# isunLt/U2MKD

Measured on AMD Instinct MI355X. Metric: LiDAR points/sec/node fwd+bwd (teacher+student+KD), 1/2/4/8 MI355X, higher is better.
Workload: dtype f32 (fp32 products emulated on the 16-bit matrix pipe: f16x2 forward / input gradient, bf16x3 weight gradient; fp32 accumulate)

## Files before the change

include/u2mkd_hip.h:

```cpp
#ifndef U2MKD_HIP_H
#define U2MKD_HIP_H

#include <stddef.h>
#include <stdint.h>

#ifdef __cplusplus
extern "C" {
#endif

typedef void *u2mkd_stream_t;

int u2mkd_version(void);
const char *u2mkd_last_error(void);
int u2mkd_stream_wait_stream(u2mkd_stream_t waiter, u2mkd_stream_t signaler);
void *u2mkd_mailbox_alloc(size_t bytes);
int u2mkd_mailbox_free(void *p);
int u2mkd_mailbox_post(const void *const *srcs, uint32_t is64, int32_t n, int64_t *slot, int64_t seq, u2mkd_stream_t s);

int u2mkd_hash(const int32_t *coords , int64_t n, int64_t *out , u2mkd_stream_t s);
int u2mkd_kernel_hash(const int32_t *coords , const int32_t *offsets , int64_t n,
                      int32_t k, int64_t *out , u2mkd_stream_t s);

size_t u2mkd_hash_table_bytes(int64_t n_refs);
int u2mkd_hash_table_build(const int64_t *refs, int64_t n_refs, void *table, u2mkd_stream_t s);
int u2mkd_hash_table_query(const void *table, int64_t n_refs, const int64_t *queries, int64_t n_q,
                           int64_t *out , u2mkd_stream_t s);
int u2mkd_hash_table_query2(const void *table, int64_t n_refs, const int64_t *queries, int64_t n_q, int64_t *out,
                            int32_t *out32, u2mkd_stream_t s);

int u2mkd_kmap_build_table(const void *table, int64_t n_refs, const int32_t *out_coords ,
                           int64_t n_out, const int32_t *offsets , int32_t k,
                           int32_t *nbr , u2mkd_stream_t s);
int u2mkd_kmap_invert(const int32_t *nbr , int64_t n_out, int32_t k, int64_t n_in,
                      int32_t *nbr_inv , u2mkd_stream_t s);
int u2mkd_kmap_sizes(const int32_t *nbr, int64_t n_out, int32_t k, int32_t *nbsizes ,
                     int32_t *block_counts , u2mkd_stream_t s);
int u2mkd_kmap_compact(const int32_t *nbr, int64_t n_out, int32_t k, const int32_t *nbsizes ,
                       int32_t *block_counts ,
                       int32_t *nbmaps , u2mkd_stream_t s);

int64_t u2mkd_pairs_capacity(int64_t n_in, int64_t n_out, int32_t k);
int u2mkd_pairs_build(const int32_t *nbr , int64_t n_out, int64_t n_in, int32_t k,
                      const int32_t *nbsizes, int32_t *block_counts, int32_t *pair_in, int32_t *pair_out,
                      int32_t *pos_out, int32_t *pos_in, int32_t *tile_k, int32_t *meta, u2mkd_stream_t s);
int u2mkd_downsample_keys(const int32_t *coords , int64_t n, int32_t sx, int32_t sy, int32_t sz,
                          int64_t *keys , u2mkd_stream_t s);
int u2mkd_downsample_keys_checked(const int32_t *coords , int64_t n, int32_t sx, int32_t sy, int32_t sz,
                                  int64_t *keys , int32_t *range_flag, u2mkd_stream_t s);
int u2mkd_unpack_keys(const int64_t *keys, int64_t n, int32_t *coords , u2mkd_stream_t s);
int u2mkd_downsample_keys_general(const int32_t *coords , int64_t n, int32_t tsx, int32_t tsy, int32_t tsz, int32_t kx,
                                  int32_t ky, int32_t kz, int32_t sx, int32_t sy, int32_t sz, const int32_t *cmin ,
                                  int32_t m, int64_t *keys , int32_t *range_flag, u2mkd_stream_t s);
int u2mkd_floor_coords(const float *pc , int64_t n, int32_t stride, int32_t *out , u2mkd_stream_t s);

int u2mkd_transpose_weights(const float *w , int32_t k, int32_t cin, int32_t cout,
                            float *wt , u2mkd_stream_t s);
int u2mkd_conv_forward(const float *in , int64_t n_in, int32_t cin, const float *wt ,
                       int32_t cout, const int32_t *nbr , int64_t n_out, int32_t k, int32_t kflip,
                       float *out , u2mkd_stream_t s);
int u2mkd_conv_forward_sorted(const float *in, int64_t n_in, int32_t cin, const float *wt, int32_t cout,
                              const int32_t *nbr_sorted , const int32_t *order ,
                              const int32_t *tile_order , int64_t n_out, int32_t k,
                              int32_t kflip, float *out , u2mkd_stream_t s);
int32_t u2mkd_conv_lk_supported(int32_t cin, int32_t cout, int32_t k);
int u2mkd_conv_forward_lk(const float *in , int64_t n_in, int32_t cin, const float *wt ,
                          int32_t cout, const int32_t *nbr , int64_t ld, int64_t n_rows, int32_t k, int32_t kflip,
                          float *out , u2mkd_stream_t s);
int32_t u2mkd_conv_tiles_supported(int32_t cin, int32_t cout, int32_t k);
int32_t u2mkd_conv_tiles_arith(int32_t cin, int32_t cout, int32_t k);
size_t u2mkd_weight_fragments_bytes(int32_t k, int32_t rows, int32_t cols, int32_t arith);
int u2mkd_weight_fragments(const float *w, int32_t k, int32_t rows, int32_t cols, int32_t transpose, int32_t arith,
                           void *wf, u2mkd_stream_t s);
int u2mkd_weight_fragments_batch(const int64_t *jobs, int32_t n_jobs, int64_t total_units, u2mkd_stream_t s);
int u2mkd_conv_forward_tiles(const float *in, int64_t n_in, int32_t cin, const void *wf, int32_t cout,
                             const int32_t *nbr_sorted , const int32_t *order ,
                             const int32_t *items ,
                             const int32_t *n_items , int64_t n_out, int32_t k,
                             int32_t kflip, int32_t arith, float *out , u2mkd_stream_t s);
int u2mkd_conv_forward_tiles_ep(const float *in, int64_t n_in, int32_t cin, const void *wf, int32_t cout,
                                const int32_t *nbr_sorted, const int32_t *order, const int32_t *items,
                                const int32_t *n_items, int64_t n_out, int32_t k, int32_t kflip, int32_t arith,
                                const float *scale , const float *shift , const float *res ,
                                int32_t relu, float *out, u2mkd_stream_t s);
int32_t u2mkd_pairs_gather_sum_stats_slab_rows(void);
int32_t u2mkd_pairs_gather_sum_stats_supported(int32_t cout);
int u2mkd_pairs_gather_sum_stats(const float *y, const int32_t *pos, int64_t n_rows, int32_t k, int32_t cout, float *out,
                                 float *partial, u2mkd_stream_t s);
int u2mkd_pairs_gather_sum_ep(const float *y, const int32_t *pos, int64_t n_rows, int32_t k, int32_t cout, const float *scale,
                              const float *shift, const float *res, int32_t relu, float *out, u2mkd_stream_t s);
int u2mkd_debug_conv_forward_sorted(const float *in, int64_t n_in, int32_t cin, const float *wt, int32_t cout,
                                    const int32_t *nbr_sorted, const int32_t *order, const int32_t *tile_order,
                                    int64_t n_out, int32_t k, int32_t kflip, int32_t variant, float *out,
                                    u2mkd_stream_t s);
int u2mkd_debug_conv_tile_pairs_stamps(const float *in, int64_t n_in, const void *wf ,
                                       const int32_t *nbr_sorted, const int32_t *order, const int32_t *items,
                                       const int32_t *n_items, int64_t n_out, int32_t k, int32_t arith, float *out,
                                       uint64_t *stamps, u2mkd_stream_t s);
int u2mkd_debug_wgrad_stamps(const float *a, const float *b, const int32_t *pairs, const int32_t *plan, int64_t n_rows,
                             int32_t k, void *workspace, uint64_t *stamps, u2mkd_stream_t s);
int u2mkd_conv_forward_pairs(const float *in, int64_t n_in, int32_t cin, const float *wt, int32_t cout,
                             const int32_t *pair_idx, const int32_t *tile_k, const int32_t *meta, int64_t capacity,
                             int32_t k, int32_t kc, float *y , u2mkd_stream_t s);
int32_t u2mkd_conv_pairs_x3_supported(int32_t cin, int32_t cout);
int u2mkd_conv_forward_pairs_x3(const float *in, int64_t n_in, int32_t cin, const void *wf, int32_t cout,
                                const int32_t *pair_idx, const int32_t *tile_k, const int32_t *meta, int64_t capacity,
                                int32_t k, float *y , u2mkd_stream_t s);
int u2mkd_linear_forward(const float *x , int64_t n, int32_t cin, const float *w , int32_t cout,
                         const float *bias , int32_t kc, float *y, u2mkd_stream_t s);
int u2mkd_linear_forward_x3(const float *x , int64_t n, int32_t cin, const void *wf, int32_t cout,
                            const float *bias , float *y , u2mkd_stream_t s);
int32_t u2mkd_conv_pairs_f16x2_supported(int32_t cin, int32_t cout);
int u2mkd_conv_forward_pairs_f16x2(const float *in, int64_t n_in, int32_t cin, const void *wf, int32_t cout,
                                    const int32_t *pair_idx, const int32_t *tile_k, const int32_t *meta, int64_t capacity,
                                    int32_t k, float *y, u2mkd_stream_t s);
int u2mkd_linear_forward_f16x2(const float *x, int64_t n, int32_t cin, const void *wf, int32_t cout, const float *bias,
                               float *y, u2mkd_stream_t s);
int u2mkd_pairs_gather_sum(const float *y, const int32_t *pos , int64_t n_rows, int32_t k, int32_t cout,
                           float *out , u2mkd_stream_t s);
int u2mkd_kmap_rowmask(const int32_t *nbr , int64_t n_out, int32_t k, int32_t *mask ,
                       u2mkd_stream_t s);
int u2mkd_conv_forward_tiles_bf16(const void *in , int64_t n_in, int32_t cin, const void *wf, int32_t cout,
                                  const int32_t *nbr_sorted, const int32_t *order, const int32_t *items,
                                  const int32_t *n_items, int64_t n_out, int32_t k, int32_t kflip,
                                  void *out , u2mkd_stream_t s);
int u2mkd_conv_wgrad_pairs_bf16(const void *a , int32_t ca, const void *b , int32_t cb,
                                const int32_t *pairs, const int32_t *plan, int64_t n_rows, int32_t k, int32_t swap,
                                void *workspace, size_t workspace_bytes, float *dw , u2mkd_stream_t s);
int u2mkd_conv_forward_tiles_f16(const void *in , int64_t n_in, int32_t cin, const void *wf, int32_t cout,
                                 const int32_t *nbr_sorted, const int32_t *order, const int32_t *items,
                                 const int32_t *n_items, int64_t n_out, int32_t k, int32_t kflip,
                                 void *out , u2mkd_stream_t s);
int u2mkd_conv_wgrad_pairs_f16(const void *a , int32_t ca, const void *b , int32_t cb,
                               const int32_t *pairs, const int32_t *plan, int64_t n_rows, int32_t k, int32_t swap,
                               void *workspace, size_t workspace_bytes, float *dw , u2mkd_stream_t s);
int u2mkd_conv_forward_pairs_f16(const void *in , int64_t n_in, int32_t cin, const void *wf, int32_t cout,
                                  const int32_t *pair_idx, const int32_t *tile_k, const int32_t *meta, int64_t capacity,
                                  int32_t k, void *y , u2mkd_stream_t s);
int u2mkd_linear_forward_f16(const void *x , int64_t n, int32_t cin, const void *wf, int32_t cout,
                             const float *bias , void *y , u2mkd_stream_t s);
int u2mkd_pairs_gather_sum_f16(const void *y , const int32_t *pos , int64_t n_rows, int32_t k,
                               int32_t cout, void *out , u2mkd_stream_t s);
int u2mkd_conv_forward_pairs_bf16(const void *in , int64_t n_in, int32_t cin, const void *wf, int32_t cout,
                                   const int32_t *pair_idx, const int32_t *tile_k, const int32_t *meta, int64_t capacity,
                                   int32_t k, void *y , u2mkd_stream_t s);
int u2mkd_linear_forward_bf16(const void *x , int64_t n, int32_t cin, const void *wf, int32_t cout,
                              const float *bias , void *y , u2mkd_stream_t s);
int u2mkd_pairs_gather_sum_bf16(const void *y , const int32_t *pos , int64_t n_rows, int32_t k,
                                int32_t cout, void *out , u2mkd_stream_t s);
size_t u2mkd_tile_schedule_workspace_bytes(int64_t n_rows);
int u2mkd_tile_schedule(const int32_t *mask , const int32_t *order , int64_t n_rows,
                        int32_t k, int32_t split0, int32_t split1, void *workspace, int32_t *tile_order,
                        int32_t *items, int32_t *n_items, u2mkd_stream_t s);
int32_t u2mkd_wgrad_plan_ints(int32_t k);
int u2mkd_wgrad_plan(const int32_t *nbsizes , int32_t k, int64_t n_rows, int32_t *plan, u2mkd_stream_t s);
size_t u2mkd_conv_wgrad_pairs_workspace_bytes(int64_t n_rows, int32_t ca, int32_t cb, int32_t k);
int u2mkd_conv_wgrad_pairs(const float *a, int32_t ca, const float *b, int32_t cb, const int32_t *pairs ,
                           const int32_t *plan, int64_t n_rows, int32_t k, int32_t swap, void *workspace,
                           size_t workspace_bytes, float *dw , u2mkd_stream_t s);

size_t u2mkd_convolution_workspace_bytes(int64_t n_in_rows, int64_t n_out_rows, int32_t cin, int32_t cout,
                                         const int32_t *nbsizes_host , int32_t k);
int u2mkd_convolution_forward(const float *in_feat , int64_t n_in_rows, int32_t cin,
                              float *out_feat , int64_t n_out_rows, int32_t cout,
                              const float *kernel , const int32_t *nbmaps ,
                              const int32_t *nbsizes_host , int32_t k, int32_t transpose, void *workspace,
                              size_t workspace_bytes, u2mkd_stream_t s);
int u2mkd_convolution_backward(const float *in_feat , int64_t n_in_rows, int32_t cin,
                               float *grad_in_feat , const float *grad_out_feat ,
                               int64_t n_out_rows, int32_t cout, const float *kernel ,
                               float *grad_kernel , const int32_t *nbmaps, const int32_t *nbsizes_host,
                               int32_t k, int32_t transpose, void *workspace, size_t workspace_bytes, u2mkd_stream_t s);

int u2mkd_count(const int32_t *idx , int64_t n, int32_t *counts , int64_t num,
                u2mkd_stream_t s);
int u2mkd_voxelize_forward(const float *feats , const int32_t *idx , const int32_t *counts ,
                           int64_t n, int64_t nv, int32_t c, float *out , u2mkd_stream_t s);
int u2mkd_voxelize_backward(const float *grad_out , const int32_t *idx, const int32_t *counts, int64_t n,
                            int64_t nv, int32_t c, float *grad_feats , u2mkd_stream_t s);
int u2mkd_devoxelize_forward(const float *feats , const int32_t *idx , const float *w ,
                             int64_t n, int32_t c, float *out , u2mkd_stream_t s);
int u2mkd_devoxelize_backward(const float *grad_out , const int32_t *idx , const float *w ,
                              int64_t n, int64_t nv, int32_t c, float *grad_feats ,
                              u2mkd_stream_t s);
int u2mkd_segment_sum(const float *src , int32_t c, const int32_t *entry_row ,
                      const float *entry_w , const int32_t *seg_offsets , int64_t nv,
                      int32_t mean, float *out , u2mkd_stream_t s);
int u2mkd_segment_mean(const float *src , int32_t c, const int32_t *entry_row ,
                       const int32_t *seg_offsets , const int32_t *counts , int64_t nv,
                       float *out , u2mkd_stream_t s);
int u2mkd_segment_mean_bf16(const void *src , int32_t c, const int32_t *entry_row ,
                            const int32_t *seg_offsets , const int32_t *counts , int64_t nv,
                            void *out , u2mkd_stream_t s);
int u2mkd_segment_mean_f16(const void *src , int32_t c, const int32_t *entry_row ,
                           const int32_t *seg_offsets , const int32_t *counts , int64_t nv,
                           void *out , u2mkd_stream_t s);
int u2mkd_voxelize_backward_bf16(const void *grad_out , const int32_t *idx, const int32_t *counts, int64_t n,
                                 int64_t nv, int32_t c, void *grad_feats , u2mkd_stream_t s);
int u2mkd_devoxelize_forward_bf16(const void *feats , const int32_t *idx , const float *w ,
                                  int64_t n, int32_t c, void *out , u2mkd_stream_t s);
int u2mkd_segment_sum_bf16(const void *src , int32_t c, const int32_t *entry_row ,
                           const float *entry_w , const int32_t *seg_offsets , int64_t nv,
                           int32_t mean, void *out , u2mkd_stream_t s);
int u2mkd_voxelize_backward_f16(const void *grad_out , const int32_t *idx, const int32_t *counts, int64_t n,
                                int64_t nv, int32_t c, void *grad_feats , u2mkd_stream_t s);
int u2mkd_devoxelize_forward_f16(const void *feats , const int32_t *idx , const float *w ,
                                 int64_t n, int32_t c, void *out , u2mkd_stream_t s);
int u2mkd_segment_sum_f16(const void *src , int32_t c, const int32_t *entry_row ,
                          const float *entry_w , const int32_t *seg_offsets , int64_t nv,
                          int32_t mean, void *out , u2mkd_stream_t s);
size_t u2mkd_csr_workspace_bytes(int64_t n_entries, int64_t nv);
int u2mkd_csr_build(const int32_t *keys , int64_t n_entries, int64_t nv, void *workspace,
                    int32_t *order , int32_t *seg , u2mkd_stream_t s);
size_t u2mkd_devoxelize_plan_workspace_bytes(int64_t n, int64_t nv);
int u2mkd_devoxelize_plan(const int32_t *idx8 , const float *w8 , int64_t n, int64_t nv, void *workspace,
                          int32_t *entry_row , float *entry_w , int32_t *seg , u2mkd_stream_t s);
int u2mkd_ti_weights(const float *coords , const int64_t *idx_kn , int64_t n,
                     float scale, float *w_n8 , int32_t *idx_n8 , u2mkd_stream_t s);

int u2mkd_up_plan(const int32_t *idx8 , int64_t n, int32_t H, int32_t W, int32_t h, int32_t w, float rh, float rw,
                  int32_t *idx_out , float *w_out , u2mkd_stream_t s);
int u2mkd_upbn_stats(const float *x, int32_t n_img, int32_t c, int32_t h, int32_t w, const float *a, const float *b,
                     const float *ay, const float *ax, int32_t rows_per_chunk, float *partial, u2mkd_stream_t s);
int u2mkd_upbn_dense_grad(const float *x, int32_t n_img, int32_t c, int32_t h, int32_t w, const float *a, const float *b,
                          const float *ay, const float *ax, const float *c0 , const float *c1 ,
                          int32_t rows_per_chunk, float *dx, u2mkd_stream_t s);

int u2mkd_up_bilinear_forward(const float *x, const float *skip , int64_t planes, int32_t h, int32_t w, int32_t H,
                              int32_t W, float rh, float rw, float *y, u2mkd_stream_t s);
int u2mkd_up_bilinear_backward(const float *g, int64_t planes, int32_t h, int32_t w, int32_t H, int32_t W, const int32_t *taps_y,
                               const float *wy, const int32_t *taps_x, const float *wx, int32_t tiled, float *dx, u2mkd_stream_t s);

int u2mkd_maxpool3s2_forward(const float *x, int64_t planes, int32_t h, int32_t w, float *y, uint8_t *code, u2mkd_stream_t s);
int u2mkd_maxpool3s2_backward(const float *dy, const uint8_t *code, int64_t planes, int32_t h, int32_t w, float *dx,
                              u2mkd_stream_t s);

int u2mkd_transpose_batched(const float *in, float *out, int32_t batch, int32_t rows, int32_t cols, u2mkd_stream_t s);
int u2mkd_transpose_batched_scaled(const float *in, float *out, int32_t batch, int32_t rows, int32_t cols, float scale,
                                   u2mkd_stream_t s);

int u2mkd_l2c_combine_forward(const float *g0, const float *g1, const float *g2, const float *g3, int32_t n_grids, int32_t n_img,
                              int32_t h, int32_t w, int32_t c, int32_t ch1, int32_t cw1, int32_t ch2, int32_t cw2, int32_t ch3,
                              int32_t cw3, float *out_rows, u2mkd_stream_t s);
int u2mkd_l2c_combine_backward(const float *g_rows, int32_t n_img, int32_t h, int32_t w, int32_t c, int32_t ch, int32_t cw,
                               float *d_grid, u2mkd_stream_t s);

int32_t u2mkd_select_mse_partials(void);
int u2mkd_select_mse_forward(const float *gathered, const float *pseudo, const uint8_t *fov, int64_t n, int32_t c, float *out,
                             float *partial, float *stats, u2mkd_stream_t s);
int u2mkd_select_mse_backward(const float *g_out, const float *g_loss, const float *stats, const float *gathered,
                              const float *pseudo, const uint8_t *fov, int64_t n, int32_t c, float *d_gathered, float *d_pseudo,
                              u2mkd_stream_t s);
int u2mkd_lovasz_errors(const float *probas, const int64_t *labels, int32_t ignore_index, int64_t n, int32_t c, float *errors,
                        double *keys, u2mkd_stream_t s);
int u2mkd_lovasz_gather(const int64_t *perm, const int64_t *labels, int32_t ignore_index, int64_t n, int32_t c,
                        int32_t *fg_sorted, u2mkd_stream_t s);
int64_t u2mkd_lovasz_partials(int64_t n, int32_t c);
int u2mkd_lovasz_terms(const int64_t *perm, const float *errors, const int64_t *csum, const int32_t *fg_sorted, int64_t n,
                       int32_t c, float *jgrad, float *partial, float *stats, u2mkd_stream_t s);
int u2mkd_lovasz_backward(const float *g_out, const float *stats, const int64_t *perm, const float *jgrad, const float *probas,
                          const int64_t *labels, int32_t ignore_index, int64_t n, int32_t c, float *d_probas, u2mkd_stream_t s);
int64_t u2mkd_ce_partials(int64_t n);
int u2mkd_ce_forward(const float *x, const int64_t *labels, int32_t ignore_index, int64_t n, int32_t c, float *lse, float *partial,
                     float *stats, u2mkd_stream_t s);
int u2mkd_ce_backward(const float *g_out, const float *stats, const float *x, const float *lse, const int64_t *labels,
                      int32_t ignore_index, int64_t n, int32_t c, float *dx, u2mkd_stream_t s);
int u2mkd_kl_forward(const float *s_logits, const float *t_logits, const int64_t *t_index, int64_t n, int32_t c, float *rows,
                     float *partial, float *stats, u2mkd_stream_t s);
int u2mkd_kl_backward(const float *g_out, const float *s_logits, const float *t_logits, const int64_t *t_index, const float *rows,
                      int64_t n, int32_t c, float *ds, u2mkd_stream_t s);
int u2mkd_c2l_plan(const float *pixel_coords, const uint8_t *mask, int32_t ncam, int64_t n, int32_t sample, int32_t h,
                   int32_t w, int32_t *idx8 , float *w8 , u2mkd_stream_t s);
int u2mkd_l2c_keys(const float *pixel_coords, const uint8_t *mask, int32_t ncam, int64_t n, int32_t sample, int64_t row0,
                   int64_t e0, int32_t ch, int32_t cw, int32_t *pix, int32_t *key_d, int32_t *key_s, int32_t *row,
                   u2mkd_stream_t s);
int u2mkd_l2c_finish(const int32_t *order_d, const int32_t *seg_d, const int32_t *order_s, const int32_t *pix,
                     const int32_t *row, int64_t n_entries, int32_t *fwd_row, float *fwd_w, int32_t *bwd_pix, float *bwd_w,
                     u2mkd_stream_t s);

int64_t u2mkd_bn_num_slabs(int64_t n);
int u2mkd_bn_train_forward(const void *x, const void *res, int32_t row_dtype, int64_t n, int32_t c, const float *gamma,
                           const float *beta, float eps, float momentum, float *running_mean, float *running_var,
                           int64_t *num_batches_tracked, int32_t relu, float *partial, float *mean ,
                           float *invstd , void *y, u2mkd_stream_t s);
int u2mkd_bn_train_forward_from_partial(const float *x, const float *res, int64_t n, int32_t c, const float *gamma,
                                        const float *beta, float eps, float momentum, float *running_mean, float *running_var,
                                        int64_t *num_batches_tracked, int32_t relu, const float *partial, int32_t slab_rows,
                                        float *mean , float *invstd , float *y, u2mkd_stream_t s);
int u2mkd_bn_eval_forward(const void *x, const void *res, int32_t row_dtype, int64_t n, int32_t c, const float *gamma,
                          const float *beta, float eps, const float *running_mean, const float *running_var, int32_t relu,
                          float *invstd , void *y, u2mkd_stream_t s);
int u2mkd_bn_backward(const void *dy, const void *x, const void *res, int32_t row_dtype, int64_t n, int32_t c,
                      const float *mean, const float *invstd, const float *gamma, const float *beta, int32_t relu,
                      int32_t training, float *partial, float *dgamma , float *dbeta , void *dx, void *dres,
                      u2mkd_stream_t s);

int u2mkd_bn_local_stats(const void *x, int32_t row_dtype, int64_t n, int32_t c, float *partial ,
                         float *stats , u2mkd_stream_t s);
int u2mkd_bn_merge_stats(const float *gathered , int32_t world, int32_t c, float eps, float momentum,
                         float *running_mean, float *running_var, float *mean , float *invstd ,
                         float *total , int64_t *num_batches_tracked, u2mkd_stream_t s);
int u2mkd_bn_apply(const void *x, const void *res, int32_t row_dtype, int64_t n, int32_t c, const float *mean,
                   const float *invstd, const float *gamma, const float *beta, int32_t relu, void *y, u2mkd_stream_t s);
int u2mkd_bn_backward_local(const void *dy, const void *x, const void *res, int32_t row_dtype, int64_t n, int32_t c,
                            const float *mean, const float *invstd, const float *gamma, const float *beta, int32_t relu,
                            float *partial , float *sums , float *keep ,
                            u2mkd_stream_t s);
int u2mkd_bn_backward_apply(const void *dy, const void *x, const void *res, int32_t row_dtype, int64_t n, int32_t c,
                            const float *total_n , const float *mean, const float *invstd, const float *gamma,
                            const float *beta, int32_t relu, const float *sums , void *dx, void *dres,
                            u2mkd_stream_t s);

int64_t u2mkd_ln_num_slabs(int64_t n, int32_t c);
int u2mkd_ln_forward(const void *x, int32_t row_dtype, int64_t n, int32_t c, const float *gamma, const float *beta, float eps,
                     float *mean , float *rstd , void *y, u2mkd_stream_t s);
int u2mkd_ln_add_forward(const void *a, const void *b, const float *w , int32_t row_dtype, int64_t n,
                         int32_t c, const float *gamma, const float *beta, float eps, float *mean ,
                         float *rstd , void *stream_out, void *y, u2mkd_stream_t s);
int u2mkd_ln_backward(const void *dy, const void *x, const void *ds , const float *w ,
                      int32_t row_dtype, int64_t n, int32_t c, const float *mean, const float *rstd, const float *gamma,
                      float *partial , float *dgamma , float *dbeta , void *dx,
                      void *db , u2mkd_stream_t s);

int64_t u2mkd_scene_num_slabs(int64_t n, int64_t nb);
int u2mkd_scene_slabs(const int32_t *seg , int64_t nb, int64_t n, int32_t *slab_seg ,
                      int32_t *slabs , int64_t nslab, u2mkd_stream_t s);
int u2mkd_gn_forward(const void *x, int32_t row_dtype, int64_t n, int32_t c, int32_t groups, const int32_t *bidx,
                     const int32_t *order, const int32_t *seg, const int32_t *slab_seg, const int32_t *slabs, int64_t nslab,
                     int64_t nb, const float *gamma, const float *beta, float eps, void *partial, float *mean, float *rstd,
                     void *y, u2mkd_stream_t s);
int u2mkd_gn_backward(const void *dy, const void *x, int32_t row_dtype, int64_t n, int32_t c, int32_t groups, const int32_t *bidx,
                      const int32_t *order, const int32_t *seg, const int32_t *slab_seg, const int32_t *slabs, int64_t nslab,
                      int64_t nb, const float *mean, const float *rstd, const float *gamma, float *partial, float *sums,
                      float *dgamma, float *dbeta, void *dx, u2mkd_stream_t s);
int u2mkd_scene_pool_forward(const void *x, int32_t row_dtype, int64_t n, int32_t c, int32_t mode, const int32_t *order,
                             const int32_t *seg, const int32_t *slab_seg, const int32_t *slabs, int64_t nslab, int64_t nb,
                             void *partial, float *out, int32_t *arg, u2mkd_stream_t s);
int u2mkd_scene_pool_backward(const float *dy, int32_t row_dtype, int64_t n, int32_t c, int32_t mode, const int32_t *bidx,
                              const int32_t *seg, const int32_t *arg, int64_t nb, void *dx, u2mkd_stream_t s);

int u2mkd_bev_plan(const int32_t *coords, int64_t n, int32_t dim, int32_t mode, int32_t hmode, int32_t s0, int32_t s1, int32_t s2,
                   int32_t a0, int32_t a1, int32_t a2, int32_t h, int32_t w, int32_t nz, int64_t *keys ,
                   int32_t *hidx , int32_t *block , u2mkd_stream_t s);
int u2mkd_bev_tables(const int32_t *group, const int32_t *hidx, int64_t n_in, int64_t n_out, int32_t nk, int32_t *nbr,
                     int32_t *nbr_inv, u2mkd_stream_t s);
int u2mkd_bev_segment_mean(const void *src, int32_t row_dtype, int64_t n_src, int32_t c, const int32_t *order, const int32_t *seg,
                           int64_t nv, void *out, u2mkd_stream_t s);
int u2mkd_bev_dense_store(const void *src, int32_t row_dtype, int64_t n_rows, int32_t c, const int32_t *seg, const int32_t *order,
                          int64_t nb, int32_t z, int32_t h, int32_t w, void *out, u2mkd_stream_t s);
int u2mkd_bev_dense_gather(const void *dout, int32_t row_dtype, int64_t n_rows, int32_t c, const int32_t *seg, const int32_t *order,
                           int64_t nb, int32_t z, int32_t h, int32_t w, void *dsrc, u2mkd_stream_t s);

int u2mkd_sptr_window_keys(const float *xyz , const int32_t *batch , int64_t n, const float *lo4,
                           const float *hi4, float sx, float sy, float sz, int64_t *keys , u2mkd_stream_t s);
size_t u2mkd_sptr_plan_prepare_workspace_bytes(void);
int u2mkd_sptr_plan_prepare(const float *xyz , const int32_t *batch , int64_t n, float cx, float cy, float cz,
                            float sx, float sy, float sz, float *sphere, float *bounds, int64_t *keys_cubic,
                            int64_t *keys_sphere, void *workspace, u2mkd_stream_t s);
int u2mkd_sptr_window_ranges(const int64_t *sorted_keys, int64_t n, int32_t *wstart , int32_t *wlen ,
                             u2mkd_stream_t s);
int u2mkd_sptr_quant_coords(const float *xyz , const int32_t *sort_idx , int64_t n, const float *lo,
                            float wx, float wy, float wz, float qx, float qy, float qz, int32_t *qc ,
                            float *radial , u2mkd_stream_t s);
int u2mkd_sptr_attention_forward(const float *q, const float *k, const float *v, const int32_t *sort_idx,
                                 const int32_t *wstart, const int32_t *wlen, const int32_t *qc, const float *radial,
                                 const float *tq, const float *tk, const float *tv, int32_t L, int32_t qgl,
                                 float split_a, int64_t n, int32_t h, int32_t hdim, float *out, float *lse,
                                 u2mkd_stream_t s);
size_t u2mkd_sptr_backward_workspace_bytes(int64_t n, int32_t h, int32_t L);
int u2mkd_sptr_attention_backward(const float *q, const float *k, const float *v, const float *out, const float *dout,
                                  const float *lse, const int32_t *sort_idx, const int32_t *wstart,
                                  const int32_t *wlen, const int32_t *qc, const float *radial, const float *tq,
                                  const float *tk, const float *tv, int32_t L, int32_t qgl, float split_a,
                                  int32_t qc_span, int64_t n, int32_t h, int32_t hdim, float *delta ,
                                  void *workspace, size_t workspace_bytes, float *dq, float *dk, float *dv, float *dtq,
                                  float *dtk, float *dtv, u2mkd_stream_t s);
int u2mkd_sptr_attention_forward_strided(const float *q, const float *k, const float *v, int64_t ld_qkv, float q_scale,
                                         const int32_t *sort_idx, const int32_t *wstart, const int32_t *wlen,
                                         const int32_t *qc, const float *radial, const float *tq, const float *tk,
                                         const float *tv, int32_t L, int32_t qgl, float split_a, int64_t n, int32_t h,
                                         int32_t hdim, float *out, int64_t ld_out, float *lse, u2mkd_stream_t s);
int u2mkd_sptr_attention_backward_strided(const float *q, const float *k, const float *v, int64_t ld_qkv, float q_scale,
                                          const float *out, const float *dout, int64_t ld_out, const float *lse,
                                          const int32_t *sort_idx, const int32_t *wstart, const int32_t *wlen,
                                          const int32_t *qc, const float *radial, const float *tq, const float *tk,
                                          const float *tv, int32_t L, int32_t qgl, float split_a, int32_t qc_span,
                                          int64_t n, int32_t h, int32_t hdim, float *delta ,
                                          void *workspace, size_t workspace_bytes, float *dq, float *dk, float *dv,
                                          int64_t ld_grad, float *dtq, float *dtk, float *dtv, u2mkd_stream_t s);
#include "u2mkd_hip_sptr_rows16.h"

int u2mkd_sptr_table_reduce(const void *workspace, int64_t n, int32_t h, int32_t L, float split_a, float *dtq, float *dtk,
                            float *dtv, u2mkd_stream_t s);

int u2mkd_sptr_quant_coords_shifted(const float *xyz , const int32_t *sort_idx , int64_t n, const float *lo,
                                    float wx, float wy, float wz, float shx, float shy, float shz, float qx, float qy,
                                    float qz, int32_t *qc , float *radial , u2mkd_stream_t s);

int u2mkd_sptr_plain_forward_strided(const float *q, const float *k, const float *v, int64_t ld_qkv, float q_scale,
                                     const int32_t *sort_idx, const int32_t *wstart, const int32_t *wlen, int64_t n,
                                     int32_t h, int32_t hdim, float *out, int64_t ld_out, float *lse, u2mkd_stream_t s);
int u2mkd_sptr_plain_backward_strided(const float *q, const float *k, const float *v, int64_t ld_qkv, float q_scale,
                                      const float *out, const float *dout, int64_t ld_out, const float *lse,
                                      const int32_t *sort_idx, const int32_t *wstart, const int32_t *wlen, int64_t n,
                                      int32_t h, int32_t hdim, float *delta , float *dq, float *dk,
                                      float *dv, int64_t ld_grad, u2mkd_stream_t s);

int u2mkd_sptr_precompute_all(int32_t N, int32_t n, uint32_t n_max, const int32_t *counts, const int32_t *offsets,
                              const int32_t *sq_offsets, int32_t *index_0_offsets, int32_t *index_1_offsets,
                              int32_t *index_0, int32_t *index_1, u2mkd_stream_t s);
int u2mkd_sptr_attention_step1_forward(int32_t N_q, int32_t N_k, int32_t M, int32_t h, int32_t hdim, uint32_t n_max,
                                       const float *q, const float *k, const int32_t *index0, const int32_t *index1,
                                       float *attn, u2mkd_stream_t s);
int u2mkd_sptr_attention_step1_backward(int32_t N, int32_t M, int32_t h, int32_t hdim, uint32_t n_max,
                                        const float *grad_out, const int32_t *index0, const int32_t *index0_offsets,
                                        const int32_t *index1, const int32_t *index1_offsets, const float *q,
                                        const float *k, float *grad_q, float *grad_k, u2mkd_stream_t s);
int u2mkd_sptr_attention_step2_forward(int32_t N, int32_t M, int32_t h, int32_t hdim, int32_t n_max, const float *attn,
                                       const float *v, const int32_t *index0_offsets, const int32_t *index1,
                                       float *output, u2mkd_stream_t s);
int u2mkd_sptr_attention_step2_backward(int32_t N, int32_t M, int32_t h, int32_t hdim, int32_t n_max,
                                        const float *grad_out, const int32_t *index0, const int32_t *index0_offsets,
                                        const int32_t *index1, const int32_t *index1_offsets, const float *attn,
                                        const float *v, float *grad_attn, float *grad_v, u2mkd_stream_t s);
int u2mkd_sptr_dot_prod_with_idx_forward(int32_t N, int32_t M, int32_t h, int32_t hdim, int32_t n_max, int32_t L,
                                         const float *q, const int32_t *index_q, const int32_t *index_q_offsets,
                                         const float *k, const int32_t *index_k, const float *table_q,
                                         const float *table_k, const int32_t *rel_idx, float *output,
                                         u2mkd_stream_t s);
int u2mkd_sptr_dot_prod_with_idx_all_forward(int32_t N, int32_t M, int32_t h, int32_t hdim, int32_t n_max, int32_t L,
                                             const float *q, const int32_t *index_q, const int32_t *index_q_offsets,
                                             const float *k, const int32_t *index_k, const float *table_q,
                                             const float *table_k, const int32_t *rel_idx, float *output,
                                             u2mkd_stream_t s);
int u2mkd_sptr_dot_prod_with_idx_backward(int32_t N, int32_t M, int32_t h, int32_t hdim, int32_t n_max, int32_t L,
                                          const float *grad_out, const float *q, const int32_t *index_q_offsets,
                                          const float *k, const int32_t *index_k_offsets, const int32_t *index_k,
                                          const float *table_q, const float *table_k, const int32_t *rel_idx,
                                          float *grad_q, float *grad_k, float *grad_table_q, float *grad_table_k,
                                          u2mkd_stream_t s);
int u2mkd_sptr_attention_step2_with_rel_pos_value_forward(int32_t N, int32_t M, int32_t h, int32_t hdim, int32_t n_max,
                                                          const float *attn, const float *v,
                                                          const int32_t *index0_offsets, const int32_t *index1,
                                                          const float *table, const int32_t *rel_idx, float *output,
                                                          u2mkd_stream_t s);
int u2mkd_sptr_attention_step2_with_rel_pos_value_backward(int32_t N, int32_t M, int32_t h, int32_t hdim, int32_t L,
                                                           int32_t n_max, const float *grad_out, const int32_t *index0,
                                                           const int32_t *index0_offsets, const int32_t *index1,
                                                           const int32_t *index1_offsets, const float *attn,
                                                           const float *v, const float *table, const int32_t *rel_idx,
                                                           float *grad_attn, float *grad_v, float *grad_table,
                                                           u2mkd_stream_t s);

size_t u2mkd_bn2d_workspace_bytes(int64_t b, int32_t c, int64_t hw);
int u2mkd_bn2d_train_forward(const float *x, const float *res, int64_t b, int32_t c, int64_t hw, const float *gamma,
                             const float *beta, float eps, float momentum, int32_t relu, float *running_mean,
                             float *running_var, int64_t *num_batches_tracked, void *workspace,
                             float *mean , float *invstd , float *y, u2mkd_stream_t s);
int u2mkd_bn2d_eval_forward(const float *x, const float *res, int64_t b, int32_t c, int64_t hw, const float *gamma,
                            const float *beta, float eps, int32_t relu, const float *running_mean,
                            const float *running_var, float *y, u2mkd_stream_t s);
int u2mkd_bn2d_backward(const float *dy, const float *x, const float *res, int64_t b, int32_t c, int64_t hw,
                        const float *mean, const float *invstd, const float *gamma, const float *beta, int32_t relu,
                        int32_t batch_stats, void *workspace, float *dgamma, float *dbeta, float *dx,
                        float *dres , u2mkd_stream_t s);

int u2mkd_bn2d_local_stats(const float *x, int64_t b, int32_t c, int64_t hw, void *workspace, float *stats ,
                           u2mkd_stream_t s);
int u2mkd_bn2d_apply(const float *x, const float *res, int64_t b, int32_t c, int64_t hw, const float *mean,
                     const float *invstd, const float *gamma, const float *beta, int32_t relu, float *y, u2mkd_stream_t s);
int u2mkd_bn2d_backward_local(const float *dy, const float *x, const float *res, int64_t b, int32_t c, int64_t hw,
                              const float *mean, const float *invstd, const float *gamma, const float *beta, int32_t relu,
                              void *workspace, float *sums , float *keep ,
                              u2mkd_stream_t s);
int u2mkd_bn2d_backward_apply(const float *dy, const float *x, const float *res, int64_t b, int32_t c, int64_t hw,
                              const float *total_n , const float *mean, const float *invstd, const float *gamma,
                              const float *beta, int32_t relu, const float *sums , float *dx,
                              float *dres , u2mkd_stream_t s);

size_t u2mkd_sptr_tiles_workspace_bytes(int64_t n, int32_t h);
int u2mkd_sptr_attention_forward_tiles(const float *q, const float *k, const float *v, int64_t ld_qkv, float q_scale,
                                       const int32_t *sort_idx, const int32_t *wstart, const int32_t *wlen, const int32_t *qc,
                                       const float *radial, const float *tq, const float *tk, const float *tv, int32_t L,
                                       int32_t qgl, float split_a, int64_t n, int32_t h, int32_t hdim, float *out, int64_t ld_out,
                                       float *lse, void *workspace, size_t workspace_bytes, u2mkd_stream_t s);

int32_t u2mkd_sgd_chunk_elements(void);
int u2mkd_sgd_batch(const int64_t *jobs, int32_t n_jobs, int64_t total_chunks, float lr, float momentum, float weight_decay,
                    int32_t nesterov, int32_t contract, u2mkd_stream_t s);
int u2mkd_grads_unscale_check(const int64_t *jobs, int32_t n_jobs, int64_t total_chunks, const float *inv_scale, float *found_inf,
                              u2mkd_stream_t s);
int u2mkd_sgd_batch_amp(const int64_t *jobs, int32_t n_jobs, int64_t total_chunks, float lr, float momentum, float weight_decay,
                        int32_t nesterov, int32_t contract, const float *grad_scale, const float *found_inf, u2mkd_stream_t s);
int u2mkd_adam_batch(const int64_t *jobs, int32_t n_jobs, int64_t total_chunks, const float *scalars, float decay, float weight_decay,
                     int32_t decoupled, float w1, float beta2, float w2, float eps, int32_t form, u2mkd_stream_t s);
int u2mkd_adam_batch_amp(const int64_t *jobs, int32_t n_jobs, int64_t total_chunks, const float *scalars, int32_t window, float decay,
                         float weight_decay, int32_t decoupled, float w1, float beta2, float w2, float eps, int32_t form,
                         const int32_t *count_in, int32_t *count_out, int32_t count_known, const float *grad_scale,
                         const float *found_inf, u2mkd_stream_t s);
int u2mkd_debug_adam_stage(int32_t stage, int32_t form, const float *a, const float *b, const float *c, float scalar, float *out,
                           int64_t n, u2mkd_stream_t s);

#ifdef __cplusplus
}
#endif
#endif
```

u2mkd_amd/_lib.py:

```python
from __future__ import annotations

import ctypes as C
import os

import torch

_HERE = os.path.dirname(os.path.abspath(__file__))
LIB_PATH = os.path.join(_HERE, 'lib', 'libu2mkd_hip%s.so' % os.environ.get('U2MKD_LIB_SUFFIX', ''))

_i32, _i64, _sz, _f32, _p = C.c_int32, C.c_int64, C.c_size_t, C.c_float, C.c_void_p

SIGNATURES = {
    'u2mkd_version': (C.c_int, []),
    'u2mkd_last_error': (C.c_char_p, []),
    'u2mkd_hash': (C.c_int, [_p, _i64, _p, _p]),
    'u2mkd_kernel_hash': (C.c_int, [_p, _p, _i64, _i32, _p, _p]),
    'u2mkd_hash_table_bytes': (_sz, [_i64]),
    'u2mkd_hash_table_build': (C.c_int, [_p, _i64, _p, _p]),
    'u2mkd_hash_table_query': (C.c_int, [_p, _i64, _p, _i64, _p, _p]),
    'u2mkd_hash_table_query2': (C.c_int, [_p, _i64, _p, _i64, _p, _p, _p]),
    'u2mkd_kmap_build_table': (C.c_int, [_p, _i64, _p, _i64, _p, _i32, _p, _p]),
    'u2mkd_kmap_invert': (C.c_int, [_p, _i64, _i32, _i64, _p, _p]),
    'u2mkd_kmap_sizes': (C.c_int, [_p, _i64, _i32, _p, _p, _p]),
    'u2mkd_kmap_compact': (C.c_int, [_p, _i64, _i32, _p, _p, _p, _p]),
    'u2mkd_downsample_keys': (C.c_int, [_p, _i64, _i32, _i32, _i32, _p, _p]),
    'u2mkd_downsample_keys_checked': (C.c_int, [_p, _i64, _i32, _i32, _i32, _p, _p, _p]),
    'u2mkd_downsample_keys_general': (C.c_int, [_p, _i64] + [_i32] * 9 + [_p, _i32, _p, _p, _p]),
    'u2mkd_floor_coords': (C.c_int, [_p, _i64, _i32, _p, _p]),
    'u2mkd_unpack_keys': (C.c_int, [_p, _i64, _p, _p]),
    'u2mkd_transpose_weights': (C.c_int, [_p, _i32, _i32, _i32, _p, _p]),
    'u2mkd_conv_forward': (C.c_int, [_p, _i64, _i32, _p, _i32, _p, _i64, _i32, _i32, _p, _p]),
    'u2mkd_conv_forward_sorted': (C.c_int, [_p, _i64, _i32, _p, _i32, _p, _p, _p, _i64, _i32, _i32, _p, _p]),
    'u2mkd_debug_conv_forward_sorted': (C.c_int, [_p, _i64, _i32, _p, _i32, _p, _p, _p, _i64, _i32, _i32, _i32, _p, _p]),
    'u2mkd_conv_lk_supported': (_i32, [_i32, _i32, _i32]),
    'u2mkd_conv_forward_lk': (C.c_int, [_p, _i64, _i32, _p, _i32, _p, _i64, _i64, _i32, _i32, _p, _p]),
    'u2mkd_stream_wait_stream': (C.c_int, [_p, _p]),
    'u2mkd_sgd_chunk_elements': (_i32, []),
    'u2mkd_sgd_batch': (C.c_int, [_p, _i32, _i64, _f32, _f32, _f32, _i32, _i32, _p]),
    'u2mkd_grads_unscale_check': (C.c_int, [_p, _i32, _i64, _p, _p, _p]),
    'u2mkd_sgd_batch_amp': (C.c_int, [_p, _i32, _i64, _f32, _f32, _f32, _i32, _i32, _p, _p, _p]),
    'u2mkd_adam_batch': (C.c_int, [_p, _i32, _i64, _p, _f32, _f32, _i32, _f32, _f32, _f32, _f32, _i32, _p]),
    'u2mkd_adam_batch_amp': (C.c_int, [_p, _i32, _i64, _p, _i32, _f32, _f32, _i32, _f32, _f32, _f32, _f32, _i32, _p, _p, _i32, _p, _p, _p]),
    'u2mkd_debug_adam_stage': (C.c_int, [_i32, _i32, _p, _p, _p, _f32, _p, _i64, _p]),
    'u2mkd_mailbox_alloc': (_p, [_sz]),
    'u2mkd_mailbox_free': (C.c_int, [_p]),
    'u2mkd_mailbox_post': (C.c_int, [_p, C.c_uint32, _i32, _p, _i64, _p]),
    'u2mkd_conv_tiles_supported': (_i32, [_i32, _i32, _i32]),
    'u2mkd_conv_tiles_arith': (_i32, [_i32, _i32, _i32]),
    'u2mkd_weight_fragments_bytes': (_sz, [_i32, _i32, _i32, _i32]),
    'u2mkd_weight_fragments': (C.c_int, [_p, _i32, _i32, _i32, _i32, _i32, _p, _p]),
    'u2mkd_weight_fragments_batch': (C.c_int, [_p, _i32, _i64, _p]),
    'u2mkd_conv_forward_tiles': (C.c_int, [_p, _i64, _i32, _p, _i32, _p, _p, _p, _p, _i64, _i32, _i32, _i32, _p, _p]),
    'u2mkd_conv_forward_tiles_ep': (C.c_int, [_p, _i64, _i32, _p, _i32, _p, _p, _p, _p, _i64, _i32, _i32, _i32, _p, _p, _p, _i32, _p, _p]),
    'u2mkd_pairs_gather_sum_ep': (C.c_int, [_p, _p, _i64, _i32, _i32, _p, _p, _p, _i32, _p, _p]),
    'u2mkd_pairs_gather_sum_stats_slab_rows': (_i32, []),
    'u2mkd_pairs_gather_sum_stats_supported': (_i32, [_i32]),
    'u2mkd_pairs_gather_sum_stats': (C.c_int, [_p, _p, _i64, _i32, _i32, _p, _p, _p]),
    'u2mkd_debug_conv_tile_pairs_stamps': (C.c_int, [_p, _i64, _p, _p, _p, _p, _p, _i64, _i32, _i32, _p, _p, _p]),
    'u2mkd_debug_wgrad_stamps': (C.c_int, [_p, _p, _p, _p, _i64, _i32, _p, _p, _p]),
    'u2mkd_conv_forward_pairs': (C.c_int, [_p, _i64, _i32, _p, _i32, _p, _p, _p, _i64, _i32, _i32, _p, _p]),
    'u2mkd_conv_pairs_x3_supported': (_i32, [_i32, _i32]),
    'u2mkd_conv_forward_pairs_x3': (C.c_int, [_p, _i64, _i32, _p, _i32, _p, _p, _p, _i64, _i32, _p, _p]),
    'u2mkd_linear_forward': (C.c_int, [_p, _i64, _i32, _p, _i32, _p, _i32, _p, _p]),
    'u2mkd_bn2d_workspace_bytes': (C.c_size_t, [_i64, _i32, _i64]),
    'u2mkd_bn2d_train_forward': (C.c_int, [_p, _p, _i64, _i32, _i64, _p, _p, C.c_float, C.c_float, _i32, _p, _p, _p, _p, _p, _p, _p, _p]),
    'u2mkd_bn2d_eval_forward': (C.c_int, [_p, _p, _i64, _i32, _i64, _p, _p, C.c_float, _i32, _p, _p, _p, _p]),
    'u2mkd_bn2d_backward': (C.c_int, [_p, _p, _p, _i64, _i32, _i64, _p, _p, _p, _p, _i32, _i32, _p, _p, _p, _p, _p, _p]),
    'u2mkd_bn2d_local_stats': (C.c_int, [_p, _i64, _i32, _i64, _p, _p, _p]),
    'u2mkd_bn2d_apply': (C.c_int, [_p, _p, _i64, _i32, _i64, _p, _p, _p, _p, _i32, _p, _p]),
    'u2mkd_bn2d_backward_local': (C.c_int, [_p, _p, _p, _i64, _i32, _i64, _p, _p, _p, _p, _i32, _p, _p, _p, _p]),
    'u2mkd_bn2d_backward_apply': (C.c_int, [_p, _p, _p, _i64, _i32, _i64, _p, _p, _p, _p, _p, _i32, _p, _p, _p, _p]),
    'u2mkd_linear_forward_x3': (C.c_int, [_p, _i64, _i32, _p, _i32, _p, _p, _p]),
    'u2mkd_conv_pairs_f16x2_supported': (_i32, [_i32, _i32]),
    'u2mkd_conv_forward_pairs_f16x2': (C.c_int, [_p, _i64, _i32, _p, _i32, _p, _p, _p, _i64, _i32, _p, _p]),
    'u2mkd_linear_forward_f16x2': (C.c_int, [_p, _i64, _i32, _p, _i32, _p, _p, _p]),
    'u2mkd_pairs_capacity': (_i64, [_i64, _i64, _i32]),
    'u2mkd_pairs_build': (C.c_int, [_p, _i64, _i64, _i32, _p, _p, _p, _p, _p, _p, _p, _p, _p]),
    'u2mkd_pairs_gather_sum': (C.c_int, [_p, _p, _i64, _i32, _i32, _p, _p]),
    'u2mkd_kmap_rowmask': (C.c_int, [_p, _i64, _i32, _p, _p]),
    'u2mkd_tile_schedule_workspace_bytes': (_sz, [_i64]),
    'u2mkd_tile_schedule': (C.c_int, [_p, _p, _i64, _i32, _i32, _i32, _p, _p, _p, _p, _p]),
    'u2mkd_wgrad_plan_ints': (_i32, [_i32]),
    'u2mkd_wgrad_plan': (C.c_int, [_p, _i32, _i64, _p, _p]),
    'u2mkd_conv_wgrad_pairs_workspace_bytes': (_sz, [_i64, _i32, _i32, _i32]),
    'u2mkd_conv_wgrad_pairs': (C.c_int, [_p, _i32, _p, _i32, _p, _p, _i64, _i32, _i32, _p, _sz, _p, _p]),
    'u2mkd_conv_forward_tiles_bf16': (C.c_int, [_p, _i64, _i32, _p, _i32, _p, _p, _p, _p, _i64, _i32, _i32, _p, _p]),
    'u2mkd_conv_forward_tiles_f16': (C.c_int, [_p, _i64, _i32, _p, _i32, _p, _p, _p, _p, _i64, _i32, _i32, _p, _p]),
    'u2mkd_conv_wgrad_pairs_bf16': (C.c_int, [_p, _i32, _p, _i32, _p, _p, _i64, _i32, _i32, _p, _sz, _p, _p]),
    'u2mkd_conv_wgrad_pairs_f16': (C.c_int, [_p, _i32, _p, _i32, _p, _p, _i64, _i32, _i32, _p, _sz, _p, _p]),
    'u2mkd_conv_forward_pairs_bf16': (C.c_int, [_p, _i64, _i32, _p, _i32, _p, _p, _p, _i64, _i32, _p, _p]),
    'u2mkd_conv_forward_pairs_f16': (C.c_int, [_p, _i64, _i32, _p, _i32, _p, _p, _p, _i64, _i32, _p, _p]),
    'u2mkd_linear_forward_bf16': (C.c_int, [_p, _i64, _i32, _p, _i32, _p, _p, _p]),
    'u2mkd_linear_forward_f16': (C.c_int, [_p, _i64, _i32, _p, _i32, _p, _p, _p]),
    'u2mkd_pairs_gather_sum_bf16': (C.c_int, [_p, _p, _i64, _i32, _i32, _p, _p]),
    'u2mkd_pairs_gather_sum_f16': (C.c_int, [_p, _p, _i64, _i32, _i32, _p, _p]),
    'u2mkd_convolution_workspace_bytes': (_sz, [_i64, _i64, _i32, _i32, _p, _i32]),
    'u2mkd_convolution_forward': (C.c_int, [_p, _i64, _i32, _p, _i64, _i32, _p, _p, _p, _i32, _i32, _p, _sz, _p]),
    'u2mkd_convolution_backward': (C.c_int, [_p, _i64, _i32, _p, _p, _i64, _i32, _p, _p, _p, _p, _i32, _i32, _p, _sz, _p]),
    'u2mkd_bn_num_slabs': (_i64, [_i64]),
    'u2mkd_bn_train_forward': (C.c_int, [_p, _p, _i32, _i64, _i32, _p, _p, _f32, _f32, _p, _p, _p, _i32, _p, _p, _p, _p, _p]),
    'u2mkd_bn_train_forward_from_partial': (C.c_int, [_p, _p, _i64, _i32, _p, _p, _f32, _f32, _p, _p, _p, _i32, _p, _i32, _p, _p, _p, _p]),
    'u2mkd_bn_eval_forward': (C.c_int, [_p, _p, _i32, _i64, _i32, _p, _p, _f32, _p, _p, _i32, _p, _p, _p]),
    'u2mkd_bn_backward': (C.c_int, [_p, _p, _p, _i32, _i64, _i32, _p, _p, _p, _p, _i32, _i32, _p, _p, _p, _p, _p, _p]),
    'u2mkd_bn_local_stats': (C.c_int, [_p, _i32, _i64, _i32, _p, _p, _p]),
    'u2mkd_bn_merge_stats': (C.c_int, [_p, _i32, _i32, _f32, _f32, _p, _p, _p, _p, _p, _p, _p]),
    'u2mkd_bn_apply': (C.c_int, [_p, _p, _i32, _i64, _i32, _p, _p, _p, _p, _i32, _p, _p]),
    'u2mkd_bn_backward_local': (C.c_int, [_p, _p, _p, _i32, _i64, _i32, _p, _p, _p, _p, _i32, _p, _p, _p, _p]),
    'u2mkd_bn_backward_apply': (C.c_int, [_p, _p, _p, _i32, _i64, _i32, _p, _p, _p, _p, _p, _i32, _p, _p, _p, _p]),
    'u2mkd_ln_num_slabs': (_i64, [_i64, _i32]),
    'u2mkd_ln_forward': (C.c_int, [_p, _i32, _i64, _i32, _p, _p, _f32, _p, _p, _p, _p]),
    'u2mkd_ln_add_forward': (C.c_int, [_p, _p, _p, _i32, _i64, _i32, _p, _p, _f32, _p, _p, _p, _p, _p]),
    'u2mkd_ln_backward': (C.c_int, [_p, _p, _p, _p, _i32, _i64, _i32, _p, _p, _p, _p, _p, _p, _p, _p, _p]),
    'u2mkd_scene_num_slabs': (_i64, [_i64, _i64]),
    'u2mkd_scene_slabs': (C.c_int, [_p, _i64, _i64, _p, _p, _i64, _p]),
    'u2mkd_gn_forward': (C.c_int, [_p, _i32, _i64, _i32, _i32, _p, _p, _p, _p, _p, _i64, _i64, _p, _p, _f32, _p, _p, _p, _p, _p]),
    'u2mkd_gn_backward': (C.c_int, [_p, _p, _i32, _i64, _i32, _i32, _p, _p, _p, _p, _p, _i64, _i64, _p, _p, _p, _p, _p, _p, _p, _p, _p]),
    'u2mkd_scene_pool_forward': (C.c_int, [_p, _i32, _i64, _i32, _i32, _p, _p, _p, _p, _i64, _i64, _p, _p, _p, _p]),
    'u2mkd_scene_pool_backward': (C.c_int, [_p, _i32, _i64, _i32, _i32, _p, _p, _p, _i64, _p, _p]),
    'u2mkd_bev_plan': (C.c_int, [_p, _i64] + [_i32] * 12 + [_p, _p, _p, _p]),
    'u2mkd_bev_tables': (C.c_int, [_p, _p, _i64, _i64, _i32, _p, _p, _p]),
    'u2mkd_bev_segment_mean': (C.c_int, [_p, _i32, _i64, _i32, _p, _p, _i64, _p, _p]),
    'u2mkd_bev_dense_store': (C.c_int, [_p, _i32, _i64, _i32, _p, _p, _i64, _i32, _i32, _i32, _p, _p]),
    'u2mkd_bev_dense_gather': (C.c_int, [_p, _i32, _i64, _i32, _p, _p, _i64, _i32, _i32, _i32, _p, _p]),
    'u2mkd_sptr_window_keys': (C.c_int, [_p, _p, _i64, _p, _p, _f32, _f32, _f32, _p, _p]),
    'u2mkd_select_mse_partials': (_i32, []),
    'u2mkd_select_mse_forward': (C.c_int, [_p, _p, _p, _i64, _i32, _p, _p, _p, _p]),
    'u2mkd_select_mse_backward': (C.c_int, [_p, _p, _p, _p, _p, _p, _i64, _i32, _p, _p, _p]),
    'u2mkd_sptr_plan_prepare_workspace_bytes': (_sz, []),
    'u2mkd_sptr_plan_prepare': (C.c_int, [_p, _p, _i64, _f32, _f32, _f32, _f32, _f32, _f32, _p, _p, _p, _p, _p, _p]),
    'u2mkd_sptr_window_ranges': (C.c_int, [_p, _i64, _p, _p, _p]),
    'u2mkd_sptr_quant_coords': (C.c_int, [_p, _p, _i64, _p, _f32, _f32, _f32, _f32, _f32, _f32, _p, _p, _p]),
    'u2mkd_sptr_attention_forward': (C.c_int, [_p, _p, _p, _p, _p, _p, _p, _p, _p, _p, _p, _i32, _i32, _f32, _i64, _i32, _i32, _p, _p, _p]),
    'u2mkd_sptr_backward_workspace_bytes': (_sz, [_i64, _i32, _i32]),
    'u2mkd_sptr_attention_backward': (C.c_int, [_p] * 14 + [_i32, _i32, _f32, _i32, _i64, _i32, _i32] + [_p, _p, _sz] + [_p] * 7),
    'u2mkd_sptr_tiles_workspace_bytes': (_sz, [_i64, _i32]),
    'u2mkd_sptr_attention_forward_tiles': (C.c_int, [_p, _p, _p, _i64, _f32] + [_p] * 8 + [_i32, _i32, _f32, _i64, _i32, _i32, _p, _i64, _p, _p, _sz, _p]),
    'u2mkd_sptr_attention_forward_strided': (C.c_int, [_p, _p, _p, _i64, _f32] + [_p] * 8 + [_i32, _i32, _f32, _i64, _i32, _i32, _p, _i64, _p, _p]),
    'u2mkd_sptr_attention_backward_strided': (C.c_int, [_p, _p, _p, _i64, _f32, _p, _p, _i64] + [_p] * 9 + [_i32, _i32, _f32, _i32, _i64, _i32, _i32]
                                              + [_p, _p, _sz] + [_p, _p, _p, _i64, _p, _p, _p, _p]),
    'u2mkd_sptr_table_reduce': (C.c_int, [_p, _i64, _i32, _i32, _f32, _p, _p, _p, _p]),
    'u2mkd_sptr_quant_coords_shifted': (C.c_int, [_p, _p, _i64, _p] + [_f32] * 9 + [_p, _p, _p]),
    'u2mkd_sptr_plain_forward_strided': (C.c_int, [_p, _p, _p, _i64, _f32, _p, _p, _p, _i64, _i32, _i32, _p, _i64, _p, _p]),
    'u2mkd_sptr_plain_backward_strided': (C.c_int, [_p, _p, _p, _i64, _f32, _p, _p, _i64, _p, _p, _p, _p, _i64, _i32, _i32,
                                                    _p, _p, _p, _p, _i64, _p]),
    'u2mkd_sptr_precompute_all': (C.c_int, [_i32, _i32, C.c_uint32] + [_p] * 8),
    'u2mkd_sptr_attention_step1_forward': (C.c_int, [_i32, _i32, _i32, _i32, _i32, C.c_uint32] + [_p] * 6),
    'u2mkd_sptr_attention_step1_backward': (C.c_int, [_i32, _i32, _i32, _i32, C.c_uint32] + [_p] * 10),
    'u2mkd_sptr_attention_step2_forward': (C.c_int, [_i32] * 5 + [_p] * 6),
    'u2mkd_sptr_attention_step2_backward': (C.c_int, [_i32] * 5 + [_p] * 10),
    'u2mkd_sptr_dot_prod_with_idx_forward': (C.c_int, [_i32] * 6 + [_p] * 10),
    'u2mkd_sptr_dot_prod_with_idx_all_forward': (C.c_int, [_i32] * 6 + [_p] * 10),
    'u2mkd_sptr_dot_prod_with_idx_backward': (C.c_int, [_i32] * 6 + [_p] * 14),
    'u2mkd_sptr_attention_step2_with_rel_pos_value_forward': (C.c_int, [_i32] * 5 + [_p] * 8),
    'u2mkd_sptr_attention_step2_with_rel_pos_value_backward': (C.c_int, [_i32] * 6 + [_p] * 13),
    'u2mkd_count': (C.c_int, [_p, _i64, _p, _i64, _p]),
    'u2mkd_voxelize_forward': (C.c_int, [_p, _p, _p, _i64, _i64, _i32, _p, _p]),
    'u2mkd_voxelize_backward': (C.c_int, [_p, _p, _p, _i64, _i64, _i32, _p, _p]),
    'u2mkd_devoxelize_forward': (C.c_int, [_p, _p, _p, _i64, _i32, _p, _p]),
    'u2mkd_devoxelize_backward': (C.c_int, [_p, _p, _p, _i64, _i64, _i32, _p, _p]),
    'u2mkd_segment_sum': (C.c_int, [_p, _i32, _p, _p, _p, _i64, _i32, _p, _p]),
    'u2mkd_voxelize_backward_bf16': (C.c_int, [_p, _p, _p, _i64, _i64, _i32, _p, _p]),
    'u2mkd_voxelize_backward_f16': (C.c_int, [_p, _p, _p, _i64, _i64, _i32, _p, _p]),
    'u2mkd_devoxelize_forward_bf16': (C.c_int, [_p, _p, _p, _i64, _i32, _p, _p]),
    'u2mkd_devoxelize_forward_f16': (C.c_int, [_p, _p, _p, _i64, _i32, _p, _p]),
    'u2mkd_segment_sum_bf16': (C.c_int, [_p, _i32, _p, _p, _p, _i64, _i32, _p, _p]),
    'u2mkd_segment_sum_f16': (C.c_int, [_p, _i32, _p, _p, _p, _i64, _i32, _p, _p]),
    'u2mkd_segment_mean': (C.c_int, [_p, _i32, _p, _p, _p, _i64, _p, _p]),
    'u2mkd_segment_mean_bf16': (C.c_int, [_p, _i32, _p, _p, _p, _i64, _p, _p]),
    'u2mkd_segment_mean_f16': (C.c_int, [_p, _i32, _p, _p, _p, _i64, _p, _p]),
    'u2mkd_c2l_plan': (C.c_int, [_p, _p, _i32, _i64, _i32, _i32, _i32, _p, _p, _p]),
    'u2mkd_l2c_keys': (C.c_int, [_p, _p, _i32, _i64, _i32, _i64, _i64, _i32, _i32, _p, _p, _p, _p, _p]),
    'u2mkd_l2c_finish': (C.c_int, [_p, _p, _p, _p, _p, _i64, _p, _p, _p, _p, _p]),
    'u2mkd_up_bilinear_forward': (C.c_int, [_p, _p, _i64, _i32, _i32, _i32, _i32, _f32, _f32, _p, _p]),
    'u2mkd_up_bilinear_backward': (C.c_int, [_p, _i64, _i32, _i32, _i32, _i32, _p, _p, _p, _p, _i32, _p, _p]),
    'u2mkd_maxpool3s2_forward': (C.c_int, [_p, _i64, _i32, _i32, _p, _p, _p]),
    'u2mkd_maxpool3s2_backward': (C.c_int, [_p, _p, _i64, _i32, _i32, _p, _p]),
    'u2mkd_transpose_batched': (C.c_int, [_p, _p, _i32, _i32, _i32, _p]),
    'u2mkd_transpose_batched_scaled': (C.c_int, [_p, _p, _i32, _i32, _i32, C.c_float, _p]),
    'u2mkd_l2c_combine_forward': (C.c_int, [_p, _p, _p, _p] + [_i32] * 11 + [_p, _p]),
    'u2mkd_l2c_combine_backward': (C.c_int, [_p] + [_i32] * 6 + [_p, _p]),
    'u2mkd_up_plan': (C.c_int, [_p, _i64, _i32, _i32, _i32, _i32, _f32, _f32, _p, _p, _p]),
    'u2mkd_upbn_stats': (C.c_int, [_p, _i32, _i32, _i32, _i32, _p, _p, _p, _p, _i32, _p, _p]),
    'u2mkd_upbn_dense_grad': (C.c_int, [_p, _i32, _i32, _i32, _i32, _p, _p, _p, _p, _p, _p, _i32, _p, _p]),
    'u2mkd_csr_workspace_bytes': (_sz, [_i64, _i64]),
    'u2mkd_lovasz_errors': (C.c_int, [_p, _p, _i32, _i64, _i32, _p, _p, _p]),
    'u2mkd_lovasz_gather': (C.c_int, [_p, _p, _i32, _i64, _i32, _p, _p]),
    'u2mkd_lovasz_partials': (_i64, [_i64, _i32]),
    'u2mkd_lovasz_terms': (C.c_int, [_p, _p, _p, _p, _i64, _i32, _p, _p, _p, _p]),
    'u2mkd_ce_partials': (_i64, [_i64]),
    'u2mkd_ce_forward': (C.c_int, [_p, _p, _i32, _i64, _i32, _p, _p, _p, _p]),
    'u2mkd_ce_backward': (C.c_int, [_p, _p, _p, _p, _p, _i32, _i64, _i32, _p, _p]),
    'u2mkd_kl_forward': (C.c_int, [_p, _p, _p, _i64, _i32, _p, _p, _p, _p]),
    'u2mkd_kl_backward': (C.c_int, [_p, _p, _p, _p, _p, _i64, _i32, _p, _p]),
    'u2mkd_lovasz_backward': (C.c_int, [_p, _p, _p, _p, _p, _p, _i32, _i64, _i32, _p, _p]),
    'u2mkd_csr_build': (C.c_int, [_p, _i64, _i64, _p, _p, _p, _p]),
    'u2mkd_devoxelize_plan_workspace_bytes': (C.c_size_t, [_i64, _i64]),
    'u2mkd_devoxelize_plan': (C.c_int, [_p, _p, _i64, _i64, _p, _p, _p, _p, _p]),
    'u2mkd_ti_weights': (C.c_int, [_p, _p, _i64, _f32, _p, _p, _p]),
}

SPTR_ROWS16_SIGNATURES = {
    name + sfx: SIGNATURES[name]
    for name in ('u2mkd_sptr_attention_forward_strided', 'u2mkd_sptr_attention_backward_strided') for sfx in ('_bf16', '_f16')}

_lib = None
_raw_stream = torch._C._cuda_getCurrentRawStream
_current_device = torch._C._cuda_getDevice


def load():
    global _lib
    if _lib is not None:
        return _lib
    if not os.path.exists(LIB_PATH):
        raise RuntimeError(
            f'{LIB_PATH} is missing: build it with `python -m u2mkd_amd.build` '
            '(u2mkd_amd has no CPU or PyTorch fallback path)')
    lib = C.CDLL(LIB_PATH)
    for name, (res, args) in list(SIGNATURES.items()) + list(SPTR_ROWS16_SIGNATURES.items()):
        fn = getattr(lib, name)
        fn.restype = res
        fn.argtypes = args
    _lib = lib
    return lib


def stream() -> int:
    return _raw_stream(_current_device())


def ptr(t):
    if t is None:
        return None
    return t.data_ptr()


_fns = {}


def call(name: str, *args):
    fn = _fns.get(name)
    if fn is None:
        fn = _fns[name] = getattr(load(), name)
    rc = fn(*args)
    if rc != 0:
        msg = load().u2mkd_last_error().decode('utf-8', 'replace')
        raise RuntimeError(f'{name} failed (rc={rc}): {msg}')


def require_cuda(*tensors):
    for t in tensors:
        if t is not None and not t.is_cuda:
            raise RuntimeError('u2mkd_amd operators run on the HIP device only (got a CPU tensor); '
                               'there is no CPU fallback')
```

u2mkd_amd/camera.py:

```python
import os

import torch
import torch.nn.functional as F
from torch import nn

__all__ = ['SwiftNetRes18', 'SwiftNetResNet', 'BNReluConv', 'BatchNorm2d', 'SyncBatchNorm2d', 'bn_act']

_HIP_BN2D = os.environ.get('U2MKD_BN2D', '1') != '0'


class _MaxPool3s2Function(torch.autograd.Function):
    @staticmethod
    def forward(ctx, x):
        from . import _lib as L
        n, c, h, w = x.shape
        oh, ow = (h - 1) // 2 + 1, (w - 1) // 2 + 1
        y = torch.empty(n, c, oh, ow, dtype=torch.float32, device=x.device)
        code = torch.empty(n, c, oh, ow, dtype=torch.uint8, device=x.device)
        L.call('u2mkd_maxpool3s2_forward', L.ptr(x), n * c, h, w, L.ptr(y), L.ptr(code), L.stream())
        ctx.save_for_backward(code)
        ctx.shape = (n, c, h, w)
        return y

    @staticmethod
    @torch.autograd.function.once_differentiable
    def backward(ctx, g):
        from . import _lib as L
        code, = ctx.saved_tensors
        n, c, h, w = ctx.shape
        dx = torch.empty(n, c, h, w, dtype=torch.float32, device=g.device)
        L.call('u2mkd_maxpool3s2_backward', L.ptr(g.contiguous()), L.ptr(code), n * c, h, w, L.ptr(dx), L.stream())
        return dx


class MaxPool3x3s2(nn.MaxPool2d):

    def __init__(self):
        super().__init__(kernel_size=3, stride=2, padding=1)

    def forward(self, x):
        if (x.is_cuda and x.dtype == torch.float32 and x.dim() == 4 and x.is_contiguous() and x.numel() and not torch.is_autocast_enabled()
                and x.shape[0] * x.shape[1] <= 65535 and x.shape[2] * x.shape[3] < 2 ** 31):
            return _MaxPool3s2Function.apply(x)
        return super().forward(x)


_UP_TAPS = {}
_UP_MODE = os.environ.get('U2MKD_UP_BILINEAR', '1')
_UP_HIP = None if _UP_MODE == 'auto' else _UP_MODE != '0'


def _up_on_hip():
    return torch.are_deterministic_algorithms_enabled() if _UP_HIP is None else _UP_HIP


def _up_taps(n_in, n_out, device):
    key = (n_in, n_out, str(device))
    if key not in _UP_TAPS:
        import numpy as np
        r = np.float32(n_in - 1) / np.float32(n_out - 1) if n_out > 1 else np.float32(0)
        src = (r * np.arange(n_out, dtype=np.float32)).astype(np.float32)
        i0 = src.astype(np.int64)
        ip = (i0 < n_in - 1).astype(np.int64)
        l1 = (src - i0.astype(np.float32)).astype(np.float32)
        l0 = (np.float32(1) - l1).astype(np.float32)
        first = np.full(n_in, n_out, np.int64)
        last = np.full(n_in, -1, np.int64)
        for idx in (i0, i0 + ip):
            np.minimum.at(first, idx, np.arange(n_out))
            np.maximum.at(last, idx, np.arange(n_out))
        cnt = np.maximum(last - first + 1, 0)
        ok = int(cnt.max()) <= 8
        taps = wts = span = None
        if ok:
            w = np.zeros((n_in, 8), np.float32)
            for o in range(n_out):
                w[i0[o], o - first[i0[o]]] += l0[o]
                w[i0[o] + ip[o], o - first[i0[o] + ip[o]]] += l1[o]
            first = np.where(cnt > 0, first, 0)
            span = {t: 1 << 30 if int(cnt.min()) == 0 else max(int(first[min(a + t, n_in) - 1] + cnt[min(a + t, n_in) - 1] - first[a]) for a in range(0, n_in, t))
                    for t in (16, 64)}
            taps = torch.tensor(np.stack([first, cnt], 1), dtype=torch.int32, device=device).contiguous()
            wts = torch.tensor(w, dtype=torch.float32, device=device).contiguous()
        _UP_TAPS[key] = (float(r), taps, wts, span)
    return _UP_TAPS[key]


class _UpBilinearFunction(torch.autograd.Function):

    @staticmethod
    def forward(ctx, x, skip, size):
        from . import _lib as L
        n, c, h, w = x.shape
        big_h, big_w = size
        rh, ty, wy, span_y = _up_taps(h, big_h, x.device)
        rw, tx, wx, span_x = _up_taps(w, big_w, x.device)
        y = torch.empty(n, c, big_h, big_w, dtype=torch.float32, device=x.device)
        L.call('u2mkd_up_bilinear_forward', L.ptr(x), L.ptr(skip), n * c, h, w, big_h, big_w, rh, rw, L.ptr(y), L.stream())
        tiled = int(span_y[16] <= 40 and span_x[64] <= 136 and n * c <= 65535)
        ctx.geom = (n, c, h, w, big_h, big_w, ty, wy, tx, wx, tiled)
        ctx.has_skip = skip is not None
        return y

    @staticmethod
    @torch.autograd.function.once_differentiable
    def backward(ctx, g):
        from . import _lib as L
        n, c, h, w, big_h, big_w, ty, wy, tx, wx, tiled = ctx.geom
        g = g.contiguous()
        dx = None
        if ctx.needs_input_grad[0]:
            dx = torch.empty(n, c, h, w, dtype=torch.float32, device=g.device)
            L.call('u2mkd_up_bilinear_backward', L.ptr(g), n * c, h, w, big_h, big_w, L.ptr(ty), L.ptr(wy), L.ptr(tx), L.ptr(wx),
                   tiled, L.ptr(dx), L.stream())
        return dx, (g if ctx.has_skip and ctx.needs_input_grad[1] else None), None


def _up(x, size, skip=None):
    size = tuple(int(v) for v in size)
    if (_up_on_hip() and x.is_cuda and x.dtype == torch.float32 and x.dim() == 4 and x.is_contiguous() and x.numel() and not torch.is_autocast_enabled()
            and x.shape[0] * x.shape[1] <= 65535 and size[0] >= x.shape[2] and size[1] >= x.shape[3] and (skip is None or (skip.dtype == x.dtype and skip.is_contiguous()
                                                                                      and skip.shape[2:] == size))):
        if _up_taps(x.shape[2], size[0], x.device)[1] is not None and _up_taps(x.shape[3], size[1], x.device)[1] is not None:
            return _UpBilinearFunction.apply(x, skip, size)
    y = F.interpolate(x, size, mode='bilinear', align_corners=True)
    return y if skip is None else y + skip


class _BatchNorm2dFunction(torch.autograd.Function):

    @staticmethod
    def forward(ctx, x, weight, bias, res, bn, relu):
        from . import _lib as L
        b, c, h, w = x.shape
        hw = h * w
        y = torch.empty_like(x)
        st = L.stream()
        batch_stats = bn.training or bn.running_mean is None
        if batch_stats:
            ws = torch.empty(max(L.load().u2mkd_bn2d_workspace_bytes(b, c, hw), 16), dtype=torch.uint8, device=x.device)
            mean = torch.empty(c, dtype=torch.float32, device=x.device)
            invstd = torch.empty_like(mean)
            track = bn.training and bn.running_mean is not None
            L.call('u2mkd_bn2d_train_forward', L.ptr(x), L.ptr(res), b, c, hw, L.ptr(weight), L.ptr(bias), bn.eps,
                   bn.momentum if track else 0.0, int(relu), L.ptr(bn.running_mean if track else None),
                   L.ptr(bn.running_var if track else None), L.ptr(bn.num_batches_tracked if track else None),
                   L.ptr(ws), L.ptr(mean), L.ptr(invstd), L.ptr(y), st)
            if track:
                torch._C._increment_version([t for t in (bn.running_mean, bn.running_var, bn.num_batches_tracked) if t is not None])
        else:
            mean, invstd = bn.running_mean, torch.rsqrt(bn.running_var + bn.eps)
            L.call('u2mkd_bn2d_eval_forward', L.ptr(x), L.ptr(res), b, c, hw, L.ptr(weight), L.ptr(bias), bn.eps, int(relu),
                   L.ptr(bn.running_mean), L.ptr(bn.running_var), L.ptr(y), st)
        ctx.save_for_backward(x, weight, bias, res, mean, invstd)
        ctx.relu, ctx.batch_stats = bool(relu), batch_stats
        return y

    @staticmethod
    def backward(ctx, dy):
        from . import _lib as L
        x, weight, bias, res, mean, invstd = ctx.saved_tensors
        b, c, h, w = x.shape
        hw = h * w
        dy = dy.contiguous()
        dx = torch.empty_like(x)
        dres = torch.empty_like(x) if res is not None else None
        dgamma = torch.empty(c, dtype=torch.float32, device=x.device)
        dbeta = torch.empty_like(dgamma)
        ws = torch.empty(max(L.load().u2mkd_bn2d_workspace_bytes(b, c, hw), 16), dtype=torch.uint8, device=x.device)
        L.call('u2mkd_bn2d_backward', L.ptr(dy), L.ptr(x), L.ptr(res), b, c, hw, L.ptr(mean), L.ptr(invstd), L.ptr(weight),
               L.ptr(bias), int(ctx.relu), int(ctx.batch_stats), L.ptr(ws), L.ptr(dgamma), L.ptr(dbeta), L.ptr(dx), L.ptr(dres),
               L.stream())
        return dx, (dgamma if weight is not None else None), (dbeta if bias is not None else None), dres, None, None


class BatchNorm2d(nn.BatchNorm2d):

    def forward(self, x, relu=False, residual=None):
        if (_HIP_BN2D and x.is_cuda and x.dtype == torch.float32 and x.dim() == 4 and x.is_contiguous() and x.numel() > 0
                and not torch.is_autocast_enabled() and (self.momentum is not None or not self.training)
                and (residual is None or (residual.dtype == x.dtype and residual.shape == x.shape))):
            if residual is not None:
                residual = residual.contiguous()
            return _BatchNorm2dFunction.apply(x, self.weight, self.bias, residual, self, relu)
        y = super().forward(x)
        if residual is not None:
            y = y + residual
        return F.relu(y) if relu else y


class _SyncBatchNorm2dFunction(torch.autograd.Function):

    @staticmethod
    def forward(ctx, x, weight, bias, res, bn, relu, group, world):
        from . import _lib as L
        from .torchsparse.nn.functional import _gather_rows, note_collective
        b, c, h, w = x.shape
        hw = h * w
        dev, st = x.device, L.stream()
        ws = torch.empty(max(L.load().u2mkd_bn2d_workspace_bytes(b, c, hw), 16), dtype=torch.uint8, device=dev)
        stats = torch.empty(2 * c + 1, dtype=torch.float32, device=dev)
        L.call('u2mkd_bn2d_local_stats', L.ptr(x), b, c, hw, L.ptr(ws), L.ptr(stats), st)
        note_collective('all_gather', stats)
        if world > 1:
            gathered = torch.empty(world, 2 * c + 1, dtype=torch.float32, device=dev)
            _gather_rows(gathered, stats, group)
        else:
            gathered = stats.view(1, -1)
        mit = torch.empty(2 * c + 1, dtype=torch.float32, device=dev)
        mean, invstd, total = mit[:c], mit[c:2 * c], mit[2 * c:]
        track = bn.running_mean is not None
        L.call('u2mkd_bn_merge_stats', L.ptr(gathered), world, c, float(bn.eps), float(bn.momentum if track else 0.0),
               L.ptr(bn.running_mean if track else None), L.ptr(bn.running_var if track else None), L.ptr(mean),
               L.ptr(invstd), L.ptr(total), L.ptr(bn.num_batches_tracked if track else None), L.stream())
        if track:
            torch._C._increment_version([t for t in (bn.running_mean, bn.running_var, bn.num_batches_tracked) if t is not None])
        y = torch.empty_like(x)
        L.call('u2mkd_bn2d_apply', L.ptr(x), L.ptr(res), b, c, hw, L.ptr(mean), L.ptr(invstd), L.ptr(weight), L.ptr(bias),
               int(relu), L.ptr(y), L.stream())
        ctx.save_for_backward(x, weight, bias, res, mean, invstd, total)
        ctx.relu, ctx.group, ctx.world = bool(relu), group, world
        return y

    @staticmethod
    def backward(ctx, dy):
        from . import _lib as L
        from .torchsparse.nn.functional import _sum_over_ranks, note_collective
        x, weight, bias, res, mean, invstd, total = ctx.saved_tensors
        b, c, h, w = x.shape
        hw = h * w
        dy = dy.contiguous()
        dev = x.device
        ws = torch.empty(max(L.load().u2mkd_bn2d_workspace_bytes(b, c, hw), 16), dtype=torch.uint8, device=dev)
        both = torch.empty(2, 2 * c, dtype=torch.float32, device=dev)
        sums, local = both[0], both[1]
        L.call('u2mkd_bn2d_backward_local', L.ptr(dy), L.ptr(x), L.ptr(res), b, c, hw, L.ptr(mean), L.ptr(invstd),
               L.ptr(weight), L.ptr(bias), int(ctx.relu), L.ptr(ws), L.ptr(sums), L.ptr(local), L.stream())
        note_collective('all_reduce', sums)
        if ctx.world > 1:
            _sum_over_ranks(sums, ctx.group)
        dx = torch.empty_like(x)
        dres = torch.empty_like(x) if res is not None else None
        L.call('u2mkd_bn2d_backward_apply', L.ptr(dy), L.ptr(x), L.ptr(res), b, c, hw, L.ptr(total), L.ptr(mean),
               L.ptr(invstd), L.ptr(weight), L.ptr(bias), int(ctx.relu), L.ptr(sums), L.ptr(dx), L.ptr(dres), L.stream())
        return (dx, local[c:] if weight is not None else None, local[:c] if bias is not None else None, dres,
                None, None, None, None)


class SyncBatchNorm2d(nn.SyncBatchNorm):

    def forward(self, x, relu=False, residual=None):
        from .torchsparse.nn.functional import _sync_group
        sync = _sync_group(self) if self.training else None
        if (sync is not None and _HIP_BN2D and x.is_cuda and x.dtype == torch.float32 and x.dim() == 4 and x.is_contiguous()
                and x.numel() > 0 and not torch.is_autocast_enabled() and self.momentum is not None
                and (residual is None or (residual.dtype == x.dtype and residual.shape == x.shape))):
            if residual is not None:
                residual = residual.contiguous()
            return _SyncBatchNorm2dFunction.apply(x, self.weight, self.bias, residual, self, relu, sync[0], sync[1])
        if (sync is None and _HIP_BN2D and x.is_cuda and x.dtype == torch.float32 and x.dim() == 4 and x.is_contiguous()
                and x.numel() > 0 and not torch.is_autocast_enabled() and (self.momentum is not None or not self.training)
                and (residual is None or (residual.dtype == x.dtype and residual.shape == x.shape))):
            if residual is not None:
                residual = residual.contiguous()
            return _BatchNorm2dFunction.apply(x, self.weight, self.bias, residual, self, relu)
        y = super().forward(x)
        if residual is not None:
            y = y + residual
        return F.relu(y) if relu else y


def bn_act(bn, x, relu=False, residual=None):
    if isinstance(bn, (BatchNorm2d, SyncBatchNorm2d)):
        return bn(x, relu, residual)
    y = bn(x)
    if residual is not None:
        y = y + residual
    return F.relu(y) if relu else y


class _Conv2dFunction(torch.autograd.Function):

    @staticmethod
    def forward(ctx, x, weight, stride, padding):
        ctx.dtypes = (x.dtype, weight.dtype)
        ctx.pid = id(weight)
        if torch.is_autocast_enabled('cuda'):
            dt = torch.get_autocast_dtype('cuda')
            x, weight = x.to(dt), weight.to(dt)
        ctx.save_for_backward(x, weight)
        ctx.conf = (stride, padding)
        with torch.autocast('cuda', enabled=False):
            return F.conv2d(x, weight, None, stride, padding)

    @staticmethod
    def backward(ctx, g):
        from . import deferred
        x, weight = ctx.saved_tensors
        stride, padding = ctx.conf
        g = g.contiguous().to(x.dtype)

        def bwd(mask):
            return torch.ops.aten.convolution_backward(g, x, weight, None, stride, padding, (1, 1), False, (0, 0), 1, mask)
        gx = bwd((True, False, False))[0].to(ctx.dtypes[0]) if ctx.needs_input_grad[0] else None
        gw = None
        if ctx.needs_input_grad[1]:
            if deferred.owned(ctx.pid):
                deferred.join()
                gw = bwd((False, True, False))[1].to(ctx.dtypes[1])
            else:
                side = deferred.side_for('camera_wgrad', g.device, owner=ctx.pid)
                with torch.cuda.stream(side):
                    gw = bwd((False, True, False))[1].to(ctx.dtypes[1])
                for t in (x, weight, g):
                    t.record_stream(side)
                gw.record_stream(torch.cuda.current_stream(g.device))
        return gx, gw, None, None


class Conv2d(nn.Conv2d):

    def forward(self, x):
        from . import deferred
        w = self.weight
        if (deferred.enabled() and deferred.overlap_ok() and x.is_cuda and torch.is_grad_enabled() and w.requires_grad and w.is_leaf and w.grad is None and self.bias is None
                and self.groups == 1 and self.dilation == (1, 1) and self.padding_mode == 'zeros'
                and not isinstance(self.padding, str) and not torch.cuda.is_current_stream_capturing()):
            return _Conv2dFunction.apply(x, w, self.stride, self.padding)
        return super().forward(x)


class BasicBlock(nn.Module):
    expansion = 1

    def __init__(self, inplanes, planes, stride=1, downsample=None):
        super().__init__()
        self.conv1 = Conv2d(inplanes, planes, 3, stride, 1, bias=False)
        self.bn1 = BatchNorm2d(planes)
        self.relu = nn.ReLU(inplace=True)
        self.conv2 = Conv2d(planes, planes, 3, 1, 1, bias=False)
        self.bn2 = BatchNorm2d(planes)
        self.downsample = downsample

    def forward(self, x):
        out = bn_act(self.bn1, self.conv1(x), relu=True)
        out = bn_act(self.bn2, self.conv2(out), relu=True, residual=x if self.downsample is None else self.downsample(x))
        return out, out


class BNReluConv(nn.Sequential):
    def __init__(self, cin, cout, k=3, bn_momentum=0.1):
        super().__init__()
        self.add_module('norm', BatchNorm2d(cin, momentum=bn_momentum))
        self.add_module('relu', nn.ReLU(inplace=True))
        self.add_module('conv', Conv2d(cin, cout, kernel_size=k, padding=k // 2, bias=False))

    def forward(self, x):
        return self.conv(bn_act(self.norm, x, relu=True))


class SpatialPyramidPooling(nn.Module):
    def __init__(self, cin, num_levels, bt_size, level_size, out_size, grids, bn_momentum):
        super().__init__()
        self.grids = grids
        self.spp = nn.Sequential()
        self.spp.add_module('spp_bn', BNReluConv(cin, bt_size, k=1, bn_momentum=bn_momentum))
        final = bt_size
        for i in range(num_levels):
            final += level_size
            self.spp.add_module('spp' + str(i), BNReluConv(bt_size, level_size, k=1, bn_momentum=bn_momentum))
        self.spp.add_module('spp_fuse', BNReluConv(final, out_size, k=1, bn_momentum=bn_momentum))

    def forward(self, x):
        h, w = x.shape[2:4]
        ar = w / h
        x = self.spp[0](x)
        levels = [x]
        for i in range(1, len(self.spp) - 1):
            grid = (self.grids[i - 1], max(1, round(ar * self.grids[i - 1])))
            levels.append(_up(self.spp[i](F.adaptive_avg_pool2d(x, grid)), (h, w)))
        return self.spp[-1](torch.cat(levels, 1))


class _Upsample(nn.Module):
    def __init__(self, cin, cskip, cout, k=3):
        super().__init__()
        self.bottleneck = BNReluConv(cskip, cin, k=1)
        self.blend_conv = BNReluConv(cin, cout, k=k)

    def forward(self, x, skip):
        skip = self.bottleneck(skip)
        return self.blend_conv(_up(x, skip.shape[2:4], skip))


class SwiftNetResNet(nn.Module):
    def __init__(self, layers=(2, 2, 2, 2), num_features=(128, 128, 128), spp_grids=(8, 4, 2, 1)):
        super().__init__()
        self.inplanes = 64
        self.img_cs = [64, 64, 128, 256, num_features[0]]
        self.conv1 = Conv2d(3, 64, kernel_size=7, stride=1, padding=3, bias=False)
        self.bn1 = BatchNorm2d(64)
        self.relu = nn.ReLU(inplace=True)
        self.maxpool = MaxPool3x3s2()
        skips = []
        self.layer1 = self._make_layer(64, layers[0])
        skips.append(self.inplanes)
        self.layer2 = self._make_layer(128, layers[1], stride=2)
        skips.append(self.inplanes)
        self.layer3 = self._make_layer(256, layers[2], stride=2)
        skips.append(self.inplanes)
        self.layer4 = self._make_layer(512, layers[3], stride=2)
        spp_size = num_features[0]
        self.spp = SpatialPyramidPooling(self.inplanes, 3, bt_size=spp_size, level_size=spp_size // 3,
                                         out_size=num_features[0], grids=spp_grids, bn_momentum=0.024 / 2)
        ups = [_Upsample(num_features[1], skips[0], num_features[2]),
               _Upsample(num_features[0], skips[1], num_features[1]),
               _Upsample(num_features[0], skips[2], num_features[0])]
        self.upsample = nn.ModuleList(list(reversed(ups)))
        self.num_features = num_features[-1]
        for m in self.modules():
            if isinstance(m, nn.Conv2d):
                nn.init.kaiming_normal_(m.weight, mode='fan_out', nonlinearity='relu')
            elif isinstance(m, nn.BatchNorm2d):
                nn.init.constant_(m.weight, 1)
                nn.init.constant_(m.bias, 0)

    def _make_layer(self, planes, blocks, stride=1):
        downsample = None
        if stride != 1 or self.inplanes != planes:
            downsample = nn.Sequential(Conv2d(self.inplanes, planes, kernel_size=1, stride=stride, bias=False),
                                       BatchNorm2d(planes))
        layers = [BasicBlock(self.inplanes, planes, stride, downsample)]
        self.inplanes = planes
        layers += [BasicBlock(planes, planes) for _ in range(1, blocks)]
        return nn.Sequential(*layers)

    @staticmethod
    def forward_resblock(x, layers):
        skip = None
        for layer in layers:
            x, skip = layer(x)
        return x, skip

    def forward_stem(self, image):
        return self.maxpool(bn_act(self.bn1, self.conv1(image), relu=True))

    def forward_down(self, image):
        x = self.forward_stem(image)
        feats = []
        for layer in (self.layer1, self.layer2, self.layer3):
            x, skip = self.forward_resblock(x, layer)
            feats.append(skip)
        x, skip = self.forward_resblock(x, self.layer4)
        feats.append(self.spp(skip))
        return feats

    def forward_up(self, features, im_size=None):
        features = features[::-1]
        x = features[0]
        for skip, up in zip(features[1:], self.upsample):
            x = up(x, skip)
        return _up(x, im_size) if im_size is not None else x

    def forward(self, image, im_size=None):
        return self.forward_up(self.forward_down(image), im_size=im_size)


def SwiftNetRes18(num_feature=(128, 128, 128), pretrained_path=None):
    model = SwiftNetResNet((2, 2, 2, 2), num_feature)
    if pretrained_path is not None:
        model.load_state_dict(torch.load(pretrained_path, map_location='cpu'), strict=False)
    return model
```

u2mkd_amd/csrc/bn2d.hip:

```cpp
#include "common.h"

namespace u2mkd {

constexpr int kB2Threads = 256;
constexpr int kB2Chunk = 8192;
constexpr int kB2ApplyChunk = 4096;

__host__ __device__ inline int b2_splits(int hw, int chunk) { return (hw + chunk - 1) / chunk; }

__device__ __forceinline__ void b2_block_sum2(float &a, float &b) {
    __shared__ float s_a[kB2Threads / 64], s_b[kB2Threads / 64];
#pragma unroll
    for (int off = 32; off >= 1; off >>= 1) {
        a += __shfl_down(a, off, 64);
        b += __shfl_down(b, off, 64);
    }
    const int lane = threadIdx.x & 63, wave = threadIdx.x >> 6;
    if (lane == 0) { s_a[wave] = a; s_b[wave] = b; }
    __syncthreads();
    if (threadIdx.x == 0) {
        a = s_a[0]; b = s_b[0];
#pragma unroll
        for (int w = 1; w < kB2Threads / 64; ++w) { a += s_a[w]; b += s_b[w]; }
    }
}

__global__ void __launch_bounds__(kB2Threads)
bn2d_stats_partial_kernel(const float *__restrict__ x, int C, int hw, int splits, float *__restrict__ partial) {
    const int c = blockIdx.y, b = blockIdx.x / splits, s = blockIdx.x - b * splits;
    const int lo = s * kB2Chunk, cnt = min(kB2Chunk, hw - lo);
    const float *p = x + ((size_t)b * C + c) * hw + lo;
    const float shift = p[0];
    float s1 = 0.f, s2 = 0.f;
    if ((hw & 3) == 0) {
        for (int e = threadIdx.x * 4; e < cnt; e += kB2Threads * 4) {
            const float4 v = *reinterpret_cast<const float4 *>(p + e);
            const float d0 = v.x - shift, d1 = v.y - shift, d2 = v.z - shift, d3 = v.w - shift;
            s1 += (d0 + d1) + (d2 + d3);
            s2 += (d0 * d0 + d1 * d1) + (d2 * d2 + d3 * d3);
        }
    } else {
        for (int e = threadIdx.x; e < cnt; e += kB2Threads) {
            const float d = p[e] - shift;
            s1 += d;
            s2 += d * d;
        }
    }
    b2_block_sum2(s1, s2);
    if (threadIdx.x == 0) {
        const float n = (float)cnt;
        float *o = partial + ((size_t)c * (gridDim.x) + blockIdx.x) * 2;
        o[0] = shift + s1 / n;
        o[1] = fmaxf(s2 - s1 * s1 / n, 0.f);
    }
}

__global__ void __launch_bounds__(64)
bn2d_stats_finalize_kernel(const float *__restrict__ partial, int np, int hw, int splits, float eps, float momentum,
                           float *__restrict__ running_mean, float *__restrict__ running_var,
                           int64_t *__restrict__ num_batches_tracked, float *__restrict__ mean_out,
                           float *__restrict__ invstd_out, float *__restrict__ m2_out = nullptr) {
    const int c = blockIdx.x, lane = threadIdx.x;
    if (num_batches_tracked && c == 0 && lane == 0) *num_batches_tracked += 1;
    float na = 0.f, mean = 0.f, m2 = 0.f;
    for (int i = lane; i < np; i += 64) {
        const int s = i % splits;
        const float nb = (float)min(kB2Chunk, hw - s * kB2Chunk);
        const float mb = partial[((size_t)c * np + i) * 2], qb = partial[((size_t)c * np + i) * 2 + 1];
        const float tot = na + nb, delta = mb - mean;
        mean += delta * (nb / tot);
        m2 += qb + delta * delta * (na * nb / tot);
        na = tot;
    }
#pragma unroll
    for (int off = 32; off >= 1; off >>= 1) {
        const float nb = __shfl_down(na, off, 64), mb = __shfl_down(mean, off, 64), qb = __shfl_down(m2, off, 64);
        if (nb != 0.f) {
            const float tot = na + nb, delta = mb - mean;
            mean += delta * (nb / tot);
            m2 += qb + delta * delta * (na * nb / tot);
            na = tot;
        }
    }
    if (lane != 0) return;
    const float var = m2 / na;
    mean_out[c] = mean;
    if (m2_out) {
        m2_out[c] = m2;
        if (c == 0) m2_out[gridDim.x] = na;
        return;
    }
    invstd_out[c] = 1.f / sqrtf(var + eps);
    if (running_mean) {
        const float unbiased = na > 1.f ? m2 / (na - 1.f) : var;
        running_mean[c] = (1.f - momentum) * running_mean[c] + momentum * mean;
        running_var[c] = (1.f - momentum) * running_var[c] + momentum * unbiased;
    }
}

__global__ void __launch_bounds__(kB2Threads)
bn2d_apply_kernel(const float *__restrict__ x, const float *__restrict__ res, int C, int hw, int asplits,
                  const float *__restrict__ mean, const float *__restrict__ invstd, const float *__restrict__ var,
                  float eps, const float *__restrict__ gamma, const float *__restrict__ beta, int relu,
                  float *__restrict__ y) {
    const int c = blockIdx.y, b = blockIdx.x / asplits, s = blockIdx.x - b * asplits;
    const int lo = s * kB2ApplyChunk, cnt = min(kB2ApplyChunk, hw - lo);
    const size_t base = ((size_t)b * C + c) * hw + lo;
    const float is = var ? 1.f / sqrtf(var[c] + eps) : invstd[c];
    const float m = mean[c], g = gamma ? gamma[c] : 1.f, bt = beta ? beta[c] : 0.f;
    auto one = [&](float v, float r) {
        const float h = (v - m) * is;
        float o = h * g + bt + r;
        return relu ? fmaxf(o, 0.f) : o;
    };
    if ((hw & 3) == 0) {
        for (int e = threadIdx.x * 4; e < cnt; e += kB2Threads * 4) {
            const float4 v = *reinterpret_cast<const float4 *>(x + base + e);
            const float4 r = res ? *reinterpret_cast<const float4 *>(res + base + e) : make_float4(0.f, 0.f, 0.f, 0.f);
            *reinterpret_cast<float4 *>(y + base + e) = make_float4(one(v.x, r.x), one(v.y, r.y), one(v.z, r.z), one(v.w, r.w));
        }
    } else {
        for (int e = threadIdx.x; e < cnt; e += kB2Threads) y[base + e] = one(x[base + e], res ? res[base + e] : 0.f);
    }
}

__global__ void __launch_bounds__(kB2Threads)
bn2d_bwd_partial_kernel(const float *__restrict__ dy, const float *__restrict__ x, const float *__restrict__ res, int C,
                        int hw, int splits, const float *__restrict__ mean, const float *__restrict__ invstd,
                        const float *__restrict__ gamma, const float *__restrict__ beta, int relu,
                        float *__restrict__ partial) {
    const int c = blockIdx.y, b = blockIdx.x / splits, s = blockIdx.x - b * splits;
    const int lo = s * kB2Chunk, cnt = min(kB2Chunk, hw - lo);
    const size_t base = ((size_t)b * C + c) * hw + lo;
    const float m = mean[c], is = invstd[c], g = gamma ? gamma[c] : 1.f, bt = beta ? beta[c] : 0.f;
    float s1 = 0.f, s2 = 0.f;
    auto one = [&](float v, float d, float r) {
        const float h = (v - m) * is;
        if (relu && h * g + bt + r <= 0.f) d = 0.f;
        s1 += d;
        s2 += d * h;
    };
    if ((hw & 3) == 0) {
        for (int e = threadIdx.x * 4; e < cnt; e += kB2Threads * 4) {
            const float4 v = *reinterpret_cast<const float4 *>(x + base + e);
            const float4 d = *reinterpret_cast<const float4 *>(dy + base + e);
            const float4 r = res ? *reinterpret_cast<const float4 *>(res + base + e) : make_float4(0.f, 0.f, 0.f, 0.f);
            one(v.x, d.x, r.x); one(v.y, d.y, r.y); one(v.z, d.z, r.z); one(v.w, d.w, r.w);
        }
    } else {
        for (int e = threadIdx.x; e < cnt; e += kB2Threads) one(x[base + e], dy[base + e], (relu && res) ? res[base + e] : 0.f);
    }
    b2_block_sum2(s1, s2);
    if (threadIdx.x == 0) {
        float *o = partial + ((size_t)c * gridDim.x + blockIdx.x) * 2;
        o[0] = s1;
        o[1] = s2;
    }
}

__global__ void __launch_bounds__(64)
bn2d_bwd_finalize_kernel(const float *__restrict__ partial, int np, float *__restrict__ dbeta, float *__restrict__ dgamma,
                         float *__restrict__ keep = nullptr) {
    const int c = blockIdx.x, lane = threadIdx.x;
    float s1 = 0.f, s2 = 0.f;
    for (int i = lane; i < np; i += 64) {
        s1 += partial[((size_t)c * np + i) * 2];
        s2 += partial[((size_t)c * np + i) * 2 + 1];
    }
#pragma unroll
    for (int off = 32; off >= 1; off >>= 1) {
        s1 += __shfl_down(s1, off, 64);
        s2 += __shfl_down(s2, off, 64);
    }
    if (lane == 0) {
        dbeta[c] = s1; dgamma[c] = s2;
        if (keep) { keep[c] = s1; keep[gridDim.x + c] = s2; }
    }
}

__global__ void __launch_bounds__(kB2Threads)
bn2d_bwd_apply_kernel(const float *__restrict__ dy, const float *__restrict__ x, const float *__restrict__ res, int C,
                      int hw, int asplits, float inv_n, const float *__restrict__ mean, const float *__restrict__ invstd,
                      const float *__restrict__ gamma, const float *__restrict__ beta, int relu,
                      const float *__restrict__ dbeta, const float *__restrict__ dgamma, float *__restrict__ dx,
                      float *__restrict__ dres, const float *__restrict__ total_n = nullptr) {
    if (total_n) inv_n = 1.f / *total_n;
    const int c = blockIdx.y, b = blockIdx.x / asplits, s = blockIdx.x - b * asplits;
    const int lo = s * kB2ApplyChunk, cnt = min(kB2ApplyChunk, hw - lo);
    const size_t base = ((size_t)b * C + c) * hw + lo;
    const float m = mean[c], is = invstd[c], g = gamma ? gamma[c] : 1.f, bt = beta ? beta[c] : 0.f;
    const float k1 = dbeta ? dbeta[c] * inv_n : 0.f, k2 = dbeta ? dgamma[c] * inv_n : 0.f, gs = g * is;
    auto one = [&](float v, float d, float r, float &dm) {
        const float h = (v - m) * is;
        if (relu && h * g + bt + r <= 0.f) d = 0.f;
        dm = d;
        return gs * (d - k1 - h * k2);
    };
    if ((hw & 3) == 0) {
        for (int e = threadIdx.x * 4; e < cnt; e += kB2Threads * 4) {
            const float4 v = *reinterpret_cast<const float4 *>(x + base + e);
            const float4 d = *reinterpret_cast<const float4 *>(dy + base + e);
            const float4 r = (relu && res) ? *reinterpret_cast<const float4 *>(res + base + e) : make_float4(0.f, 0.f, 0.f, 0.f);
            float4 o, dm;
            o.x = one(v.x, d.x, r.x, dm.x); o.y = one(v.y, d.y, r.y, dm.y);
            o.z = one(v.z, d.z, r.z, dm.z); o.w = one(v.w, d.w, r.w, dm.w);
            *reinterpret_cast<float4 *>(dx + base + e) = o;
            if (dres) *reinterpret_cast<float4 *>(dres + base + e) = dm;
        }
    } else {
        for (int e = threadIdx.x; e < cnt; e += kB2Threads) {
            float dm;
            dx[base + e] = one(x[base + e], dy[base + e], (relu && res) ? res[base + e] : 0.f, dm);
            if (dres) dres[base + e] = dm;
        }
    }
}

static bool b2_shape_ok(int64_t b, int32_t c, int64_t hw) {
    return b > 0 && c > 0 && hw > 0 && c <= 65535 && hw < ((int64_t)1 << 30) &&
           b * b2_splits((int)hw, kB2ApplyChunk) < ((int64_t)1 << 31);
}

}

using namespace u2mkd;

extern "C" {

size_t u2mkd_bn2d_workspace_bytes(int64_t b, int32_t c, int64_t hw) {
    if (b <= 0 || c <= 0 || hw <= 0) return 0;
    return (size_t)c * b * b2_splits((int)hw, kB2Chunk) * 2 * sizeof(float);
}

int u2mkd_bn2d_train_forward(const float *x, const float *res, int64_t b, int32_t c, int64_t hw, const float *gamma,
                             const float *beta, float eps, float momentum, int32_t relu, float *running_mean,
                             float *running_var, int64_t *num_batches_tracked, void *workspace, float *mean, float *invstd,
                             float *y, u2mkd_stream_t s) {
    U2_REQUIRE(x && workspace && mean && invstd && y, "u2mkd_bn2d_train_forward: null pointer");
    U2_REQUIRE(b2_shape_ok(b, c, hw), "u2mkd_bn2d_train_forward: shape [%lld, %d, %lld] out of range", (long long)b, c, (long long)hw);
    U2_REQUIRE(b * hw > 1, "u2mkd_bn2d_train_forward: more than one value per channel is needed in training mode");
    const int splits = b2_splits((int)hw, kB2Chunk), asplits = b2_splits((int)hw, kB2ApplyChunk);
    float *partial = reinterpret_cast<float *>(workspace);
    hipLaunchKernelGGL(bn2d_stats_partial_kernel, dim3((unsigned)(splits * b), (unsigned)c), dim3(kB2Threads), 0, as_stream(s), x,
                       c, (int)hw, splits, partial);
    hipLaunchKernelGGL(bn2d_stats_finalize_kernel, dim3((unsigned)c), dim3(64), 0, as_stream(s), partial, (int)(splits * b),
                       (int)hw, splits, eps, momentum, running_mean, running_var, num_batches_tracked, mean, invstd);
    hipLaunchKernelGGL(bn2d_apply_kernel, dim3((unsigned)(asplits * b), (unsigned)c), dim3(kB2Threads), 0, as_stream(s), x, res, c,
                       (int)hw, asplits, mean, invstd, nullptr, eps, gamma, beta, relu, y);
    return check_launch("u2mkd_bn2d_train_forward");
}

int u2mkd_bn2d_eval_forward(const float *x, const float *res, int64_t b, int32_t c, int64_t hw, const float *gamma,
                            const float *beta, float eps, int32_t relu, const float *running_mean, const float *running_var,
                            float *y, u2mkd_stream_t s) {
    U2_REQUIRE(x && running_mean && running_var && y, "u2mkd_bn2d_eval_forward: null pointer");
    U2_REQUIRE(b2_shape_ok(b, c, hw), "u2mkd_bn2d_eval_forward: shape [%lld, %d, %lld] out of range", (long long)b, c, (long long)hw);
    const int asplits = b2_splits((int)hw, kB2ApplyChunk);
    hipLaunchKernelGGL(bn2d_apply_kernel, dim3((unsigned)(asplits * b), (unsigned)c), dim3(kB2Threads), 0, as_stream(s), x, res, c,
                       (int)hw, asplits, running_mean, nullptr, running_var, eps, gamma, beta, relu, y);
    return check_launch("u2mkd_bn2d_eval_forward");
}

int u2mkd_bn2d_backward(const float *dy, const float *x, const float *res, int64_t b, int32_t c, int64_t hw,
                        const float *mean, const float *invstd, const float *gamma, const float *beta, int32_t relu,
                        int32_t batch_stats, void *workspace, float *dgamma, float *dbeta, float *dx, float *dres,
                        u2mkd_stream_t s) {
    U2_REQUIRE(dy && x && mean && invstd && workspace && dgamma && dbeta && dx, "u2mkd_bn2d_backward: null pointer");
    U2_REQUIRE(b2_shape_ok(b, c, hw), "u2mkd_bn2d_backward: shape [%lld, %d, %lld] out of range", (long long)b, c, (long long)hw);
    const int splits = b2_splits((int)hw, kB2Chunk), asplits = b2_splits((int)hw, kB2ApplyChunk);
    float *partial = reinterpret_cast<float *>(workspace);
    hipLaunchKernelGGL(bn2d_bwd_partial_kernel, dim3((unsigned)(splits * b), (unsigned)c), dim3(kB2Threads), 0, as_stream(s), dy, x,
                       res, c, (int)hw, splits, mean, invstd, gamma, beta, relu, partial);
    hipLaunchKernelGGL(bn2d_bwd_finalize_kernel, dim3((unsigned)c), dim3(64), 0, as_stream(s), partial, (int)(splits * b), dbeta,
                       dgamma);
    hipLaunchKernelGGL(bn2d_bwd_apply_kernel, dim3((unsigned)(asplits * b), (unsigned)c), dim3(kB2Threads), 0, as_stream(s), dy, x,
                       res, c, (int)hw, asplits, 1.f / (float)(b * hw), mean, invstd, gamma, beta, relu, batch_stats ? dbeta : nullptr,
                       batch_stats ? dgamma : nullptr, dx, dres);
    return check_launch("u2mkd_bn2d_backward");
}

int u2mkd_bn2d_local_stats(const float *x, int64_t b, int32_t c, int64_t hw, void *workspace, float *stats ,
                           u2mkd_stream_t s) {
    U2_REQUIRE(x && workspace && stats, "u2mkd_bn2d_local_stats: null pointer");
    U2_REQUIRE(b2_shape_ok(b, c, hw), "u2mkd_bn2d_local_stats: shape [%lld, %d, %lld] out of range", (long long)b, c, (long long)hw);
    const int splits = b2_splits((int)hw, kB2Chunk);
    float *partial = reinterpret_cast<float *>(workspace);
    hipLaunchKernelGGL(bn2d_stats_partial_kernel, dim3((unsigned)(splits * b), (unsigned)c), dim3(kB2Threads), 0, as_stream(s), x,
                       c, (int)hw, splits, partial);
    hipLaunchKernelGGL(bn2d_stats_finalize_kernel, dim3((unsigned)c), dim3(64), 0, as_stream(s), partial, (int)(splits * b),
                       (int)hw, splits, 0.f, 0.f, (float *)nullptr, (float *)nullptr, (int64_t *)nullptr, stats, (float *)nullptr,
                       stats + c);
    return check_launch("u2mkd_bn2d_local_stats");
}

int u2mkd_bn2d_apply(const float *x, const float *res, int64_t b, int32_t c, int64_t hw, const float *mean,
                     const float *invstd, const float *gamma, const float *beta, int32_t relu, float *y, u2mkd_stream_t s) {
    U2_REQUIRE(x && mean && invstd && y, "u2mkd_bn2d_apply: null pointer");
    U2_REQUIRE(b2_shape_ok(b, c, hw), "u2mkd_bn2d_apply: shape [%lld, %d, %lld] out of range", (long long)b, c, (long long)hw);
    const int asplits = b2_splits((int)hw, kB2ApplyChunk);
    hipLaunchKernelGGL(bn2d_apply_kernel, dim3((unsigned)(asplits * b), (unsigned)c), dim3(kB2Threads), 0, as_stream(s), x, res, c,
                       (int)hw, asplits, mean, invstd, nullptr, 0.f, gamma, beta, relu, y);
    return check_launch("u2mkd_bn2d_apply");
}

int u2mkd_bn2d_backward_local(const float *dy, const float *x, const float *res, int64_t b, int32_t c, int64_t hw,
                              const float *mean, const float *invstd, const float *gamma, const float *beta, int32_t relu,
                              void *workspace, float *sums ,
                              float *keep ,
                              u2mkd_stream_t s) {
    U2_REQUIRE(dy && x && mean && invstd && workspace && sums, "u2mkd_bn2d_backward_local: null pointer");
    U2_REQUIRE(b2_shape_ok(b, c, hw), "u2mkd_bn2d_backward_local: shape [%lld, %d, %lld] out of range", (long long)b, c, (long long)hw);
    const int splits = b2_splits((int)hw, kB2Chunk);
    float *partial = reinterpret_cast<float *>(workspace);
    hipLaunchKernelGGL(bn2d_bwd_partial_kernel, dim3((unsigned)(splits * b), (unsigned)c), dim3(kB2Threads), 0, as_stream(s), dy, x,
                       res, c, (int)hw, splits, mean, invstd, gamma, beta, relu, partial);
    hipLaunchKernelGGL(bn2d_bwd_finalize_kernel, dim3((unsigned)c), dim3(64), 0, as_stream(s), partial, (int)(splits * b), sums,
                       sums + c, keep);
    return check_launch("u2mkd_bn2d_backward_local");
}

int u2mkd_bn2d_backward_apply(const float *dy, const float *x, const float *res, int64_t b, int32_t c, int64_t hw,
                              const float *total_n, const float *mean, const float *invstd, const float *gamma,
                              const float *beta, int32_t relu, const float *sums , float *dx,
                              float *dres, u2mkd_stream_t s) {
    U2_REQUIRE(dy && x && total_n && mean && invstd && sums && dx, "u2mkd_bn2d_backward_apply: null pointer");
    U2_REQUIRE(b2_shape_ok(b, c, hw), "u2mkd_bn2d_backward_apply: shape [%lld, %d, %lld] out of range", (long long)b, c, (long long)hw);
    const int asplits = b2_splits((int)hw, kB2ApplyChunk);
    hipLaunchKernelGGL(bn2d_bwd_apply_kernel, dim3((unsigned)(asplits * b), (unsigned)c), dim3(kB2Threads), 0, as_stream(s), dy, x,
                       res, c, (int)hw, asplits, 0.f, mean, invstd, gamma, beta, relu, sums, sums + c, dx, dres, total_n);
    return check_launch("u2mkd_bn2d_backward_apply");
}

}
```

u2mkd_amd/csrc/pixhead.hip:

```cpp
#include "common.h"

namespace u2mkd {

constexpr int kPhThreads = 256;

__global__ void __launch_bounds__(kPhThreads)
up_plan_kernel(const int32_t *__restrict__ idx8, int64_t n, int H, int W, int h, int w, float rh, float rw,
               int32_t *__restrict__ idx_out, float *__restrict__ w_out) {
#pragma clang fp contract(off)
    const int64_t t = (int64_t)blockIdx.x * blockDim.x + threadIdx.x;
    if (t >= n * 4) return;
    const int64_t f = idx8[(t >> 2) * 8 + (t & 3)];
    int32_t *oi = idx_out + t * 8;
    float *ow = w_out + t * 8;
#pragma unroll
    for (int s = 0; s < 8; ++s) { oi[s] = -1; ow[s] = 0.f; }
    if (f < 0) return;
    const int64_t hw_full = (int64_t)H * W;
    const int64_t img = f / hw_full;
    const int rem = (int)(f - img * hw_full);
    const int y = rem / W, x = rem - y * W;
    const float h1r = rh * (float)y, w1r = rw * (float)x;
    const int h1 = (int)h1r, w1 = (int)w1r;
    const int h1p = h1 < h - 1 ? 1 : 0, w1p = w1 < w - 1 ? 1 : 0;
    const float hl1 = h1r - (float)h1, wl1 = w1r - (float)w1;
    const float hl0 = 1.f - hl1, wl0 = 1.f - wl1;
    const int64_t base = img * (int64_t)h * w;
    oi[0] = (int32_t)(base + (int64_t)h1 * w + w1);                 ow[0] = hl0 * wl0;
    oi[1] = (int32_t)(base + (int64_t)h1 * w + w1 + w1p);           ow[1] = hl0 * wl1;
    oi[2] = (int32_t)(base + (int64_t)(h1 + h1p) * w + w1);         ow[2] = hl1 * wl0;
    oi[3] = (int32_t)(base + (int64_t)(h1 + h1p) * w + w1 + w1p);   ow[3] = hl1 * wl1;
}

__device__ __forceinline__ void stage_rows(const float *__restrict__ xp, int h, int w, int r0, int r1, float k0, float *s_x) {
    const int n = (r1 - r0 + 2) * w;
    for (int e = threadIdx.x; e < n; e += blockDim.x) {
        const int r = r0 - 1 + e / w;
        s_x[e] = (r >= 0 && r < h) ? xp[(int64_t)r * w + (e % w)] - k0 : 0.f;
    }
    __syncthreads();
}

__device__ __forceinline__ float stencil_lds(const float *s_x, int li, int j, int i, int h, int w, const float *__restrict__ ay,
                                             const float *__restrict__ ax) {
    const float al = j > 0 ? ax[j] : 0.f, am = ax[w + j], au = j < w - 1 ? ax[2 * w + j] : 0.f;
    const int jl = j > 0 ? j - 1 : j, ju = j < w - 1 ? j + 1 : j;
    float t = 0.f;
#pragma unroll
    for (int di = 0; di < 3; ++di) {
        const float *row = s_x + (li + di) * w;
        t += ay[di * h + i] * (al * row[jl] + am * row[j] + au * row[ju]);
    }
    return t;
}

__global__ void __launch_bounds__(kPhThreads)
upbn_stats_kernel(const float *__restrict__ X, int C, int h, int w, const float *__restrict__ a, const float *__restrict__ b,
                  const float *__restrict__ ay, const float *__restrict__ ax, int rows_per_chunk,
                  float *__restrict__ partial) {
    extern __shared__ __attribute__((aligned(16))) float s_x[];
    __shared__ float red[2][kPhThreads / 64];
    const int plane = blockIdx.x, chunk = blockIdx.y;
    const int c = plane % C;
    const float k0 = X[(int64_t)c * h * w];
    const float *xp = X + (int64_t)plane * h * w;
    const int r0 = chunk * rows_per_chunk, r1 = min(h, r0 + rows_per_chunk);
    stage_rows(xp, h, w, r0, r1, k0, s_x);
    float s1 = 0.f, s2 = 0.f;
    for (int e = threadIdx.x; e < (r1 - r0) * w; e += kPhThreads) {
        const int li = e / w, j = e - li * w, i = r0 + li;
        const float xc = s_x[(li + 1) * w + j];
        s1 += a[i] * b[j] * xc;
        s2 += xc * stencil_lds(s_x, li, j, i, h, w, ay, ax);
    }
#pragma unroll
    for (int off = 32; off >= 1; off >>= 1) {
        s1 += __shfl_down(s1, off);
        s2 += __shfl_down(s2, off);
    }
    if ((threadIdx.x & 63) == 0) {
        red[0][threadIdx.x >> 6] = s1;
        red[1][threadIdx.x >> 6] = s2;
    }
    __syncthreads();
    if (threadIdx.x == 0) {
        float *o = partial + ((int64_t)plane * gridDim.y + chunk) * 2;
        o[0] = red[0][0] + red[0][1] + red[0][2] + red[0][3];
        o[1] = red[1][0] + red[1][1] + red[1][2] + red[1][3];
    }
}

__global__ void __launch_bounds__(kPhThreads)
upbn_dense_grad_kernel(const float *__restrict__ X, int C, int h, int w, const float *__restrict__ a,
                       const float *__restrict__ b, const float *__restrict__ ay, const float *__restrict__ ax,
                       const float *__restrict__ c0, const float *__restrict__ c1, int rows_per_chunk,
                       float *__restrict__ dX) {
    extern __shared__ __attribute__((aligned(16))) float s_x[];
    const int plane = blockIdx.x, chunk = blockIdx.y;
    const int c = plane % C;
    const float *xp = X + (int64_t)plane * h * w;
    float *dp = dX + (int64_t)plane * h * w;
    const int r0 = chunk * rows_per_chunk, r1 = min(h, r0 + rows_per_chunk);
    stage_rows(xp, h, w, r0, r1, 0.f, s_x);
    const float k0c = c0[c], k1c = c1[c];
    for (int e = threadIdx.x; e < (r1 - r0) * w; e += kPhThreads) {
        const int li = e / w, j = e - li * w, i = r0 + li;
        dp[(int64_t)i * w + j] = k0c * a[i] * b[j] + k1c * stencil_lds(s_x, li, j, i, h, w, ay, ax);
    }
}

constexpr int kTrTile = 64;
__global__ void __launch_bounds__(256)
transpose_kernel(const float *__restrict__ in, float *__restrict__ out, int rows, int cols, float scale = 1.f) {
    __shared__ float tile[kTrTile][kTrTile + 1];
    const size_t plane = (size_t)blockIdx.z * rows * cols;
    const int c0 = blockIdx.x * kTrTile, r0 = blockIdx.y * kTrTile;
    const int tx = threadIdx.x & 63, ty = threadIdx.x >> 6;
#pragma unroll
    for (int k = 0; k < kTrTile; k += 4) {
        const int r = r0 + ty + k, c = c0 + tx;
        if (r < rows && c < cols) tile[ty + k][tx] = in[plane + (size_t)r * cols + c];
    }
    __syncthreads();
#pragma unroll
    for (int k = 0; k < kTrTile; k += 4) {
        const int c = c0 + ty + k, r = r0 + tx;
        if (c < cols && r < rows) out[plane + (size_t)c * rows + r] = tile[tx][ty + k] * scale;
    }
}

struct L2cGrids {
    const float *g[4];
    int ch[4], cw[4];
    float ry[4], rx[4];
    int n;
};

__device__ __forceinline__ void l2c_taps(int d, float r, int n_src, int &i0, int &i1, float &f) {
    const float s = r * (float)d;
    i0 = (int)s;
    if (i0 > n_src - 1) i0 = n_src - 1;
    f = s - (float)i0;
    i1 = i0 + (i0 < n_src - 1 ? 1 : 0);
}

__global__ void __launch_bounds__(256)
l2c_combine_rows_kernel(L2cGrids G, int n_img, int H, int W, int c4, float4 *__restrict__ out) {
    const int64_t t = (int64_t)blockIdx.x * 256 + threadIdx.x;
    if (t >= (int64_t)n_img * H * W * c4) return;
    const int c = (int)(t % c4);
    const int64_t pix = t / c4;
    const int x = (int)(pix % W), y = (int)((pix / W) % H), img = (int)(pix / ((int64_t)W * H));
    float4 acc = reinterpret_cast<const float4 *>(G.g[0])[t];
#pragma unroll
    for (int s = 1; s < 4; ++s) {
        if (s >= G.n) break;
        int y0, y1, x0, x1;
        float fy, fx;
        l2c_taps(y, G.ry[s], G.ch[s], y0, y1, fy);
        l2c_taps(x, G.rx[s], G.cw[s], x0, x1, fx);
        const float4 *g = reinterpret_cast<const float4 *>(G.g[s]) + (int64_t)img * G.ch[s] * G.cw[s] * c4 + c;
        const float4 a = g[((int64_t)y0 * G.cw[s] + x0) * c4], b = g[((int64_t)y0 * G.cw[s] + x1) * c4];
        const float4 d = g[((int64_t)y1 * G.cw[s] + x0) * c4], e = g[((int64_t)y1 * G.cw[s] + x1) * c4];
        const float w00 = (1.f - fy) * (1.f - fx), w01 = (1.f - fy) * fx, w10 = fy * (1.f - fx), w11 = fy * fx;
        acc.x += w00 * a.x + w01 * b.x + w10 * d.x + w11 * e.x;
        acc.y += w00 * a.y + w01 * b.y + w10 * d.y + w11 * e.y;
        acc.z += w00 * a.z + w01 * b.z + w10 * d.z + w11 * e.z;
        acc.w += w00 * a.w + w01 * b.w + w10 * d.w + w11 * e.w;
    }
    out[t] = acc;
}

__global__ void __launch_bounds__(256)
l2c_combine_rows_bwd_kernel(const float4 *__restrict__ g, int n_img, int H, int W, int c4, int ch, int cw, float ry, float rx,
                            float4 *__restrict__ d) {
    const int64_t t = (int64_t)blockIdx.x * 256 + threadIdx.x;
    if (t >= (int64_t)n_img * ch * cw * c4) return;
    const int c = (int)(t % c4);
    const int64_t cell = t / c4;
    const int j = (int)(cell % cw), i = (int)((cell / cw) % ch), img = (int)(cell / ((int64_t)cw * ch));
    int ylo = 0, yhi = H - 1, xlo = 0, xhi = W - 1;
    if (ry > 0.f) { ylo = max(0, (int)floorf((float)(i - 1) / ry) - 1); yhi = min(H - 1, (int)ceilf((float)(i + 1) / ry) + 1); }
    if (rx > 0.f) { xlo = max(0, (int)floorf((float)(j - 1) / rx) - 1); xhi = min(W - 1, (int)ceilf((float)(j + 1) / rx) + 1); }
    float4 acc = make_float4(0.f, 0.f, 0.f, 0.f);
    for (int y = ylo; y <= yhi; ++y) {
        int y0, y1;
        float fy;
        l2c_taps(y, ry, ch, y0, y1, fy);
        const float wy = (y0 == i ? 1.f - fy : 0.f) + (y1 == i ? fy : 0.f);
        if (wy == 0.f) continue;
        const float4 *row = g + ((int64_t)img * H + y) * W * c4 + c;
        for (int x = xlo; x <= xhi; ++x) {
            int x0, x1;
            float fx;
            l2c_taps(x, rx, cw, x0, x1, fx);
            const float w = wy * ((x0 == j ? 1.f - fx : 0.f) + (x1 == j ? fx : 0.f));
            if (w == 0.f) continue;
            const float4 v = row[(int64_t)x * c4];
            acc.x += w * v.x; acc.y += w * v.y; acc.z += w * v.z; acc.w += w * v.w;
        }
    }
    d[t] = acc;
}

__global__ void __launch_bounds__(256)
maxpool3s2_fwd_kernel(const float *__restrict__ x, int h, int w, int oh, int ow, float *__restrict__ y,
                      uint8_t *__restrict__ code) {
    const uint32_t pix = blockIdx.x * blockDim.x + threadIdx.x;
    if (pix >= (uint32_t)(oh * ow)) return;
    const int oy = (int)(pix / (uint32_t)ow), ox = (int)(pix - (uint32_t)oy * (uint32_t)ow);
    const int64_t plane = blockIdx.y;
    const int64_t e = plane * oh * ow + pix;
    const float *xp = x + plane * (int64_t)h * w;
    const int y0 = 2 * oy - 1, x0 = 2 * ox - 1;
    float best = -INFINITY;
    int bc = 0;
    bool first = true;
#pragma unroll
    for (int dy = 0; dy < 3; ++dy) {
        const int yy = y0 + dy;
        if (yy < 0 || yy >= h) continue;
#pragma unroll
        for (int dx = 0; dx < 3; ++dx) {
            const int xx = x0 + dx;
            if (xx < 0 || xx >= w) continue;
            const float v = xp[(int64_t)yy * w + xx];
            if (first || v > best || v != v) { best = v; bc = dy * 3 + dx; first = false; }
        }
    }
    y[e] = best;
    code[e] = (uint8_t)bc;
}

__global__ void __launch_bounds__(256)
maxpool3s2_bwd_kernel(const float *__restrict__ dy, const uint8_t *__restrict__ code, int h, int w, int oh, int ow,
                      float *__restrict__ dx) {
    const uint32_t pix = blockIdx.x * blockDim.x + threadIdx.x;
    if (pix >= (uint32_t)(h * w)) return;
    const int yy = (int)(pix / (uint32_t)w), xx = (int)(pix - (uint32_t)yy * (uint32_t)w);
    const int64_t plane = blockIdx.y;
    const int64_t e = plane * h * w + pix;
    const float *gp = dy + plane * (int64_t)oh * ow;
    const uint8_t *cp = code + plane * (int64_t)oh * ow;
    float g = 0.f;
    const int oy0 = yy >> 1, oy1 = (yy + 1) >> 1, ox0 = xx >> 1, ox1 = (xx + 1) >> 1;
#pragma unroll
    for (int a = 0; a < 2; ++a) {
        const int oy = a ? oy1 : oy0;
        if ((a && oy1 == oy0) || oy >= oh) continue;
        const int dyw = yy - (2 * oy - 1);
#pragma unroll
        for (int b = 0; b < 2; ++b) {
            const int ox = b ? ox1 : ox0;
            if ((b && ox1 == ox0) || ox >= ow) continue;
            const int dxw = xx - (2 * ox - 1);
            if (cp[(int64_t)oy * ow + ox] == dyw * 3 + dxw) g += gp[(int64_t)oy * ow + ox];
        }
    }
    dx[e] = g;
}

__global__ void __launch_bounds__(256)
maxpool3s2_bwd4_kernel(const float *__restrict__ dy, const uint8_t *__restrict__ code, int h, int w, int oh, int ow,
                       float *__restrict__ dx) {
    const int w4 = w >> 2;
    const uint32_t q = blockIdx.x * blockDim.x + threadIdx.x;
    if (q >= (uint32_t)(h * w4)) return;
    const int yy = (int)(q / (uint32_t)w4), x0 = 4 * (int)(q - (uint32_t)yy * (uint32_t)w4);
    const int64_t plane = blockIdx.y;
    const float *gp = dy + plane * (int64_t)oh * ow;
    const uint8_t *cp = code + plane * (int64_t)oh * ow;
    const int oy0 = yy >> 1, oy1 = (yy + 1) >> 1, oxb = x0 >> 1;
    float g[4] = {0.f, 0.f, 0.f, 0.f};
#pragma unroll
    for (int a = 0; a < 2; ++a) {
        const int oy = a ? oy1 : oy0;
        if ((a && oy1 == oy0) || oy >= oh) continue;
        const int dyw = yy - (2 * oy - 1);
#pragma unroll
        for (int b = 0; b < 3; ++b) {
            const int ox = oxb + b;
            if (ox >= ow) continue;
            const int sel = (int)cp[(int64_t)oy * ow + ox] - 3 * dyw;
            const float v = gp[(int64_t)oy * ow + ox];
            const int col = 2 * ox - 1 + sel - x0;
#pragma unroll
            for (int i = 0; i < 4; ++i) g[i] += (sel >= 0 && sel < 3 && col == i) ? v : 0.f;
        }
    }
    *reinterpret_cast<float4 *>(dx + plane * (int64_t)h * w + (int64_t)yy * w + x0) = make_float4(g[0], g[1], g[2], g[3]);
}

__device__ __forceinline__ void up_source(float scale, int dst, int &i0, float &lambda1) {
#pragma clang fp contract(off)
    const float src = scale * (float)dst;
    i0 = (int)src;
    lambda1 = src - (float)i0;
}

__global__ void __launch_bounds__(256)
up_bilinear_fwd_kernel(const float *__restrict__ x, const float *__restrict__ skip, int64_t total, int h, int w, int H, int W,
                       float rh, float rw, float *__restrict__ y) {
    const int64_t e = (int64_t)blockIdx.x * blockDim.x + threadIdx.x;
    if (e >= total) return;
    const int ox = (int)(e % W);
    const int64_t r = e / W;
    const int oy = (int)(r % H);
    const int64_t plane = r / H;
    int h1, w1;
    float h1l, w1l;
    up_source(rh, oy, h1, h1l);
    up_source(rw, ox, w1, w1l);
    const int h1p = h1 < h - 1 ? 1 : 0, w1p = w1 < w - 1 ? 1 : 0;
    const float h0l = 1.f - h1l, w0l = 1.f - w1l;
    const float *xp = x + plane * (int64_t)h * w + (int64_t)h1 * w + w1;
    float v = h0l * (w0l * xp[0] + w1l * xp[w1p]) + h1l * (w0l * xp[(int64_t)h1p * w] + w1l * xp[(int64_t)h1p * w + w1p]);
    if (skip) v += skip[e];
    y[e] = v;
}

constexpr int kUpTaps = 8;
__global__ void __launch_bounds__(256)
up_bilinear_bwd_kernel(const float *__restrict__ g, int64_t total_in, int h, int w, int H, int W, const int2 *__restrict__ ty,
                       const float *__restrict__ wy, const int2 *__restrict__ tx, const float *__restrict__ wx,
                       float *__restrict__ dx) {
    const int64_t e = (int64_t)blockIdx.x * blockDim.x + threadIdx.x;
    if (e >= total_in) return;
    const int j = (int)(e % w);
    const int64_t r = e / w;
    const int i = (int)(r % h);
    const int64_t plane = r / h;
    const float *gp = g + plane * (int64_t)H * W;
    const int2 ry = ty[i], rx = tx[j];
    float acc = 0.f;
    for (int a = 0; a < ry.y; ++a) {
        const float *row = gp + (int64_t)(ry.x + a) * W + rx.x;
        float t = 0.f;
        for (int b = 0; b < rx.y; ++b) t += wx[j * kUpTaps + b] * row[b];
        acc += wy[i * kUpTaps + a] * t;
    }
    dx[e] = acc;
}

constexpr int kUpTi = 16, kUpTj = 64, kUpLr = 40, kUpLc = 136;
__global__ void __launch_bounds__(256)
up_bilinear_bwd_tiled_kernel(const float *__restrict__ g, int h, int w, int H, int W, const int2 *__restrict__ ty,
                             const float *__restrict__ wy, const int2 *__restrict__ tx, const float *__restrict__ wx,
                             float *__restrict__ dx) {
    __shared__ float win[kUpLr][kUpLc + 1];
    const int j0 = blockIdx.x * kUpTj, i0 = blockIdx.y * kUpTi;
    const int64_t plane = blockIdx.z;
    const int i1 = min(i0 + kUpTi, h) - 1, j1 = min(j0 + kUpTj, w) - 1;
    const int r_lo = ty[i0].x, r_hi = ty[i1].x + ty[i1].y, c_lo = tx[j0].x, c_hi = tx[j1].x + tx[j1].y;
    const int nr = r_hi - r_lo, nc = c_hi - c_lo;
    const float *gp = g + plane * (int64_t)H * W;
    for (int rr = threadIdx.x / 64; rr < nr; rr += 4)
        for (int cc = threadIdx.x % 64; cc < nc; cc += 64) win[rr][cc] = gp[(int64_t)(r_lo + rr) * W + c_lo + cc];
    __syncthreads();
    const int j = j0 + threadIdx.x % 64;
    if (j > j1) return;
    const int2 rx = tx[j];
    float wxj[kUpTaps];
#pragma unroll
    for (int b = 0; b < kUpTaps; ++b) wxj[b] = wx[j * kUpTaps + b];
    const int cb = rx.x - c_lo;
    for (int i = i0 + threadIdx.x / 64; i <= i1; i += 4) {
        const int2 ry = ty[i];
        float acc = 0.f;
        for (int a = 0; a < ry.y; ++a) {
            const float *row = &win[ry.x - r_lo + a][cb];
            float t = 0.f;
#pragma unroll
            for (int b = 0; b < kUpTaps; ++b)
                if (b < rx.y) t += wxj[b] * row[b];
            acc += wy[i * kUpTaps + a] * t;
        }
        dx[plane * (int64_t)h * w + (int64_t)i * w + j] = acc;
    }
}

}

using namespace u2mkd;

extern "C" {

int u2mkd_up_plan(const int32_t *idx8, int64_t n, int32_t H, int32_t W, int32_t h, int32_t w, float rh, float rw,
                  int32_t *idx_out, float *w_out, u2mkd_stream_t s) {
    if (n == 0) return 0;
    U2_REQUIRE(idx8 && idx_out && w_out, "u2mkd_up_plan: null pointer");
    U2_REQUIRE(H > 0 && W > 0 && h > 0 && w > 0 && h <= H && w <= W, "u2mkd_up_plan: bad sizes %dx%d <- %dx%d", H, W, h, w);
    U2_REQUIRE(n * 4 < ((int64_t)1 << 31), "u2mkd_up_plan: more than 2^31 samples");
    hipLaunchKernelGGL(up_plan_kernel, dim3((unsigned)ceil_div(n * 4, kPhThreads)), dim3(kPhThreads), 0, as_stream(s), idx8, n,
                       H, W, h, w, rh, rw, idx_out, w_out);
    return check_launch("u2mkd_up_plan");
}

int u2mkd_upbn_stats(const float *x, int32_t n_img, int32_t c, int32_t h, int32_t w, const float *a, const float *b,
                     const float *ay, const float *ax, int32_t rows_per_chunk, float *partial, u2mkd_stream_t s) {
    U2_REQUIRE(x && a && b && ay && ax && partial, "u2mkd_upbn_stats: null pointer");
    U2_REQUIRE(n_img > 0 && c > 0 && h > 0 && w > 0 && rows_per_chunk > 0, "u2mkd_upbn_stats: bad shape");
    const int chunks = (int)ceil_div(h, rows_per_chunk);
    U2_REQUIRE((int64_t)n_img * c < ((int64_t)1 << 31) && chunks <= 65535, "u2mkd_upbn_stats: grid too large");
    const size_t lds = (size_t)(rows_per_chunk + 2) * w * sizeof(float);
    U2_REQUIRE(lds <= 60 * 1024, "u2mkd_upbn_stats: %d rows of %d floats do not fit the LDS stage", rows_per_chunk + 2, w);
    hipLaunchKernelGGL(upbn_stats_kernel, dim3((unsigned)(n_img * c), (unsigned)chunks), dim3(kPhThreads), lds, as_stream(s), x,
                       c, h, w, a, b, ay, ax, rows_per_chunk, partial);
    return check_launch("u2mkd_upbn_stats");
}

int u2mkd_upbn_dense_grad(const float *x, int32_t n_img, int32_t c, int32_t h, int32_t w, const float *a, const float *b,
                          const float *ay, const float *ax, const float *c0, const float *c1, int32_t rows_per_chunk,
                          float *dx, u2mkd_stream_t s) {
    U2_REQUIRE(x && a && b && ay && ax && c0 && c1 && dx, "u2mkd_upbn_dense_grad: null pointer");
    U2_REQUIRE(n_img > 0 && c > 0 && h > 0 && w > 0 && rows_per_chunk > 0, "u2mkd_upbn_dense_grad: bad shape");
    const int chunks = (int)ceil_div(h, rows_per_chunk);
    const size_t lds = (size_t)(rows_per_chunk + 2) * w * sizeof(float);
    U2_REQUIRE(lds <= 60 * 1024 && chunks <= 65535, "u2mkd_upbn_dense_grad: %d rows of %d floats do not fit the LDS stage",
               rows_per_chunk + 2, w);
    hipLaunchKernelGGL(upbn_dense_grad_kernel, dim3((unsigned)(n_img * c), (unsigned)chunks), dim3(kPhThreads), lds, as_stream(s),
                       x, c, h, w, a, b, ay, ax, c0, c1, rows_per_chunk, dx);
    return check_launch("u2mkd_upbn_dense_grad");
}

int u2mkd_transpose_batched(const float *in, float *out, int32_t batch, int32_t rows, int32_t cols, u2mkd_stream_t s) {
    if (batch == 0 || rows == 0 || cols == 0) return 0;
    U2_REQUIRE(in && out && batch > 0 && rows > 0 && cols > 0, "u2mkd_transpose_batched: bad arguments");
    U2_REQUIRE(batch <= 65535 && ceil_div(rows, kTrTile) <= 65535, "u2mkd_transpose_batched: grid too large");
    hipLaunchKernelGGL(transpose_kernel, dim3((unsigned)ceil_div(cols, kTrTile), (unsigned)ceil_div(rows, kTrTile), (unsigned)batch),
                       dim3(256), 0, as_stream(s), in, out, rows, cols);
    return check_launch("u2mkd_transpose_batched");
}

int u2mkd_transpose_batched_scaled(const float *in, float *out, int32_t batch, int32_t rows, int32_t cols, float scale,
                                   u2mkd_stream_t s) {
    if (batch == 0 || rows == 0 || cols == 0) return 0;
    U2_REQUIRE(in && out && batch > 0 && rows > 0 && cols > 0, "u2mkd_transpose_batched_scaled: bad arguments");
    U2_REQUIRE(batch <= 65535 && ceil_div(rows, kTrTile) <= 65535, "u2mkd_transpose_batched_scaled: grid too large");
    hipLaunchKernelGGL(transpose_kernel, dim3((unsigned)ceil_div(cols, kTrTile), (unsigned)ceil_div(rows, kTrTile), (unsigned)batch),
                       dim3(256), 0, as_stream(s), in, out, rows, cols, scale);
    return check_launch("u2mkd_transpose_batched_scaled");
}

static float l2c_ratio(int n_src, int n_dst) { return n_dst > 1 ? (float)(n_src - 1) / (float)(n_dst - 1) : 0.f; }

int u2mkd_l2c_combine_forward(const float *g0, const float *g1, const float *g2, const float *g3, int32_t n_grids, int32_t n_img,
                              int32_t h, int32_t w, int32_t c, int32_t ch1, int32_t cw1, int32_t ch2, int32_t cw2, int32_t ch3,
                              int32_t cw3, float *out_rows, u2mkd_stream_t s) {
    U2_REQUIRE(n_grids >= 1 && n_grids <= 4 && c > 0 && c % 4 == 0 && n_img > 0 && h > 0 && w > 0,
               "u2mkd_l2c_combine_forward: %d grids of %d channels (1..4 grids, channels a multiple of 4)", n_grids, c);
    U2_REQUIRE(g0 && out_rows && (n_grids < 2 || g1) && (n_grids < 3 || g2) && (n_grids < 4 || g3), "u2mkd_l2c_combine_forward: null pointer");
    L2cGrids G;
    const float *gp[4] = {g0, g1, g2, g3};
    const int chs[4] = {h, ch1, ch2, ch3}, cws[4] = {w, cw1, cw2, cw3};
    for (int i = 0; i < 4; ++i) {
        G.g[i] = gp[i]; G.ch[i] = chs[i]; G.cw[i] = cws[i];
        G.ry[i] = l2c_ratio(chs[i], h); G.rx[i] = l2c_ratio(cws[i], w);
        U2_REQUIRE(i >= n_grids || (chs[i] > 0 && cws[i] > 0 && chs[i] <= h && cws[i] <= w), "u2mkd_l2c_combine_forward: grid %d is %dx%d", i, chs[i], cws[i]);
    }
    G.n = n_grids;
    const int64_t total = (int64_t)n_img * h * w * (c / 4);
    hipLaunchKernelGGL(l2c_combine_rows_kernel, dim3((unsigned)ceil_div(total, 256)), dim3(256), 0, as_stream(s), G, n_img, h, w,
                       c / 4, reinterpret_cast<float4 *>(out_rows));
    return check_launch("u2mkd_l2c_combine_forward");
}

int u2mkd_l2c_combine_backward(const float *g_rows, int32_t n_img, int32_t h, int32_t w, int32_t c, int32_t ch, int32_t cw,
                               float *d_grid, u2mkd_stream_t s) {
    U2_REQUIRE(g_rows && d_grid && c > 0 && c % 4 == 0 && n_img > 0 && h > 0 && w > 0 && ch > 0 && cw > 0 && ch <= h && cw <= w,
               "u2mkd_l2c_combine_backward: bad arguments");
    const int64_t total = (int64_t)n_img * ch * cw * (c / 4);
    hipLaunchKernelGGL(l2c_combine_rows_bwd_kernel, dim3((unsigned)ceil_div(total, 256)), dim3(256), 0, as_stream(s),
                       reinterpret_cast<const float4 *>(g_rows), n_img, h, w, c / 4, ch, cw, l2c_ratio(ch, h), l2c_ratio(cw, w),
                       reinterpret_cast<float4 *>(d_grid));
    return check_launch("u2mkd_l2c_combine_backward");
}

int u2mkd_maxpool3s2_forward(const float *x, int64_t planes, int32_t h, int32_t w, float *y, uint8_t *code, u2mkd_stream_t s) {
    if (planes == 0) return 0;
    U2_REQUIRE(x && y && code && planes > 0 && h > 0 && w > 0, "u2mkd_maxpool3s2_forward: bad arguments");
    const int oh = (h + 2 - 3) / 2 + 1, ow = (w + 2 - 3) / 2 + 1;
    U2_REQUIRE(planes <= 65535 && (int64_t)h * w < ((int64_t)1 << 31), "u2mkd_maxpool3s2_forward: at most 65535 planes of < 2^31 pixels");
    hipLaunchKernelGGL(maxpool3s2_fwd_kernel, dim3((unsigned)ceil_div((int64_t)oh * ow, 256), (unsigned)planes), dim3(256), 0,
                       as_stream(s), x, h, w, oh, ow, y, code);
    return check_launch("u2mkd_maxpool3s2_forward");
}

int u2mkd_maxpool3s2_backward(const float *dy, const uint8_t *code, int64_t planes, int32_t h, int32_t w, float *dx,
                              u2mkd_stream_t s) {
    if (planes == 0) return 0;
    U2_REQUIRE(dy && code && dx && planes > 0 && h > 0 && w > 0, "u2mkd_maxpool3s2_backward: bad arguments");
    const int oh = (h + 2 - 3) / 2 + 1, ow = (w + 2 - 3) / 2 + 1;
    U2_REQUIRE(planes <= 65535 && (int64_t)h * w < ((int64_t)1 << 31), "u2mkd_maxpool3s2_backward: at most 65535 planes of < 2^31 pixels");
    if (w % 4 == 0 && (reinterpret_cast<uintptr_t>(dx) & 15) == 0)
        hipLaunchKernelGGL(maxpool3s2_bwd4_kernel, dim3((unsigned)ceil_div((int64_t)h * (w / 4), 256), (unsigned)planes), dim3(256), 0,
                           as_stream(s), dy, code, h, w, oh, ow, dx);
    else
        hipLaunchKernelGGL(maxpool3s2_bwd_kernel, dim3((unsigned)ceil_div((int64_t)h * w, 256), (unsigned)planes), dim3(256), 0,
                           as_stream(s), dy, code, h, w, oh, ow, dx);
    return check_launch("u2mkd_maxpool3s2_backward");
}

int u2mkd_up_bilinear_forward(const float *x, const float *skip, int64_t planes, int32_t h, int32_t w, int32_t H, int32_t W,
                              float rh, float rw, float *y, u2mkd_stream_t s) {
    if (planes == 0) return 0;
    U2_REQUIRE(x && y && planes > 0 && h > 0 && w > 0 && H > 0 && W > 0, "u2mkd_up_bilinear_forward: bad arguments");
    const int64_t total = planes * H * W;
    hipLaunchKernelGGL(up_bilinear_fwd_kernel, dim3((unsigned)ceil_div(total, 256)), dim3(256), 0, as_stream(s), x, skip, total, h,
                       w, H, W, rh, rw, y);
    return check_launch("u2mkd_up_bilinear_forward");
}

int u2mkd_up_bilinear_backward(const float *g, int64_t planes, int32_t h, int32_t w, int32_t H, int32_t W, const int32_t *taps_y,
                               const float *wy, const int32_t *taps_x, const float *wx, int32_t tiled, float *dx, u2mkd_stream_t s) {
    if (planes == 0) return 0;
    U2_REQUIRE(g && taps_y && wy && taps_x && wx && dx && planes > 0 && h > 0 && w > 0 && H > 0 && W > 0,
               "u2mkd_up_bilinear_backward: bad arguments");
    U2_REQUIRE(!tiled || planes <= 65535, "u2mkd_up_bilinear_backward: the tiled form takes at most 65535 planes");
    const int64_t total = planes * h * w;
    if (tiled) {
        hipLaunchKernelGGL(up_bilinear_bwd_tiled_kernel, dim3((unsigned)ceil_div(w, kUpTj), (unsigned)ceil_div(h, kUpTi), (unsigned)planes),
                           dim3(256), 0, as_stream(s), g, h, w, H, W, reinterpret_cast<const int2 *>(taps_y), wy,
                           reinterpret_cast<const int2 *>(taps_x), wx, dx);
        return check_launch("u2mkd_up_bilinear_backward");
    }
    hipLaunchKernelGGL(up_bilinear_bwd_kernel, dim3((unsigned)ceil_div(total, 256)), dim3(256), 0, as_stream(s), g, total, h, w, H,
                       W, reinterpret_cast<const int2 *>(taps_y), wy, reinterpret_cast<const int2 *>(taps_x), wx, dx);
    return check_launch("u2mkd_up_bilinear_backward");
}

}
```

Measured before the change: 1.198 million.

## Fuse stem BatchNorm+ReLU with 3x3 stride-2 maxpool forward and backward

Adds kernels that apply BN normalisation and ReLU inside the maxpool window read, so the full-resolution activated stem tensor is never written. In backward, the pool gradient scatter is folded into the BN backward partial and apply kernels through a templated gradient accessor that gathers from the pooled gradient and argmax codes. This removes a full-size intermediate write and read plus separate pool kernels, in exchange for recomputing BN on overlapping windows and doing more index arithmetic per element in the backward. Sync-BN and non-sync paths are both wired, and the pool helpers are shared with the existing pixhead kernels.

```diff
diff --git a/include/u2mkd_hip.h b/include/u2mkd_hip.h
--- a/include/u2mkd_hip.h
+++ b/include/u2mkd_hip.h
@@ -477,6 +477,26 @@
                               const float *beta, int32_t relu, const float *sums , float *dx,
                               float *dres , u2mkd_stream_t s);
 
+int u2mkd_bn2d_pool_train_forward(const float *x, int64_t b, int32_t c, int32_t h, int32_t w, const float *gamma,
+                                  const float *beta, float eps, float momentum, float *running_mean, float *running_var,
+                                  int64_t *num_batches_tracked, void *workspace, float *mean ,
+                                  float *invstd , float *y, uint8_t *code, u2mkd_stream_t s);
+int u2mkd_bn2d_pool_eval_forward(const float *x, int64_t b, int32_t c, int32_t h, int32_t w, const float *gamma,
+                                 const float *beta, float eps, const float *running_mean, const float *running_var, float *y,
+                                 uint8_t *code, u2mkd_stream_t s);
+int u2mkd_bn2d_pool_apply(const float *x, int64_t b, int32_t c, int32_t h, int32_t w, const float *mean, const float *invstd,
+                          const float *gamma, const float *beta, float *y, uint8_t *code, u2mkd_stream_t s);
+int u2mkd_bn2d_pool_backward(const float *g, const uint8_t *code, const float *x, int64_t b, int32_t c, int32_t h, int32_t w,
+                             const float *mean, const float *invstd, const float *gamma, const float *beta,
+                             int32_t batch_stats, void *workspace, float *dgamma, float *dbeta, float *dx, u2mkd_stream_t s);
+int u2mkd_bn2d_pool_backward_local(const float *g, const uint8_t *code, const float *x, int64_t b, int32_t c, int32_t h,
+                                   int32_t w, const float *mean, const float *invstd, const float *gamma, const float *beta,
+                                   void *workspace, float *sums , float *keep , u2mkd_stream_t s);
+int u2mkd_bn2d_pool_backward_apply(const float *g, const uint8_t *code, const float *x, int64_t b, int32_t c, int32_t h,
+                                   int32_t w, const float *total_n , const float *mean, const float *invstd,
+                                   const float *gamma, const float *beta, const float *sums ,
+                                   float *dx, u2mkd_stream_t s);
+
 size_t u2mkd_sptr_tiles_workspace_bytes(int64_t n, int32_t h);
 int u2mkd_sptr_attention_forward_tiles(const float *q, const float *k, const float *v, int64_t ld_qkv, float q_scale,
                                        const int32_t *sort_idx, const int32_t *wstart, const int32_t *wlen, const int32_t *qc,
diff --git a/u2mkd_amd/_lib.py b/u2mkd_amd/_lib.py
--- a/u2mkd_amd/_lib.py
+++ b/u2mkd_amd/_lib.py
@@ -70,7 +70,13 @@
     'u2mkd_bn2d_apply': (C.c_int, [_p, _p, _i64, _i32, _i64, _p, _p, _p, _p, _i32, _p, _p]),
     'u2mkd_bn2d_backward_local': (C.c_int, [_p, _p, _p, _i64, _i32, _i64, _p, _p, _p, _p, _i32, _p, _p, _p, _p]),
     'u2mkd_bn2d_backward_apply': (C.c_int, [_p, _p, _p, _i64, _i32, _i64, _p, _p, _p, _p, _p, _i32, _p, _p, _p, _p]),
-    'u2mkd_linear_forward_x3': (C.c_int, [_p, _i64, _i32, _p, _i32, _p, _p, _p]),
+    'u2mkd_bn2d_pool_train_forward': (C.c_int, [_p, _i64, _i32, _i32, _i32, _p, _p, C.c_float, C.c_float, _p, _p, _p, _p, _p, _p, _p, _p, _p]),
+    'u2mkd_bn2d_pool_eval_forward': (C.c_int, [_p, _i64, _i32, _i32, _i32, _p, _p, C.c_float, _p, _p, _p, _p, _p]),
+    'u2mkd_bn2d_pool_apply': (C.c_int, [_p, _i64, _i32, _i32, _i32, _p, _p, _p, _p, _p, _p, _p]),
+    'u2mkd_bn2d_pool_backward': (C.c_int, [_p, _p, _p, _i64, _i32, _i32, _i32, _p, _p, _p, _p, _i32, _p, _p, _p, _p, _p]),
+    'u2mkd_bn2d_pool_backward_local': (C.c_int, [_p, _p, _p, _i64, _i32, _i32, _i32, _p, _p, _p, _p, _p, _p, _p, _p]),
+    'u2mkd_bn2d_pool_backward_apply': (C.c_int, [_p, _p, _p, _i64, _i32, _i32, _i32, _p, _p, _p, _p, _p, _p, _p, _p]),
+    'u2mkd_linear_forward_x3':(C.c_int, [_p, _i64, _i32, _p, _i32, _p, _p, _p]),
     'u2mkd_conv_pairs_f16x2_supported': (_i32, [_i32, _i32]),
     'u2mkd_conv_forward_pairs_f16x2': (C.c_int, [_p, _i64, _i32, _p, _i32, _p, _p, _p, _i64, _i32, _p, _p]),
     'u2mkd_linear_forward_f16x2': (C.c_int, [_p, _i64, _i32, _p, _i32, _p, _p, _p]),
diff --git a/u2mkd_amd/camera.py b/u2mkd_amd/camera.py
--- a/u2mkd_amd/camera.py
+++ b/u2mkd_amd/camera.py
@@ -4,7 +4,7 @@
 import torch.nn.functional as F
 from torch import nn
 
-__all__ = ['SwiftNetRes18', 'SwiftNetResNet', 'BNReluConv', 'BatchNorm2d', 'SyncBatchNorm2d', 'bn_act']
+__all__ = ['SwiftNetRes18', 'SwiftNetResNet', 'BNReluConv', 'BatchNorm2d', 'SyncBatchNorm2d', 'bn_act', 'bn_relu_pool']
 
 _HIP_BN2D = os.environ.get('U2MKD_BN2D', '1') != '0'
 
@@ -268,6 +268,126 @@
         if residual is not None:
             y = y + residual
         return F.relu(y) if relu else y
+
+
+def _pool_out(x):
+    b, c, h, w = x.shape
+    y = torch.empty(b, c, (h - 1) // 2 + 1, (w - 1) // 2 + 1, dtype=torch.float32, device=x.device)
+    return y, torch.empty(y.shape, dtype=torch.uint8, device=x.device)
+
+
+class _BNReluPoolFunction(torch.autograd.Function):
+
+    @staticmethod
+    def forward(ctx, x, weight, bias, bn):
+        from . import _lib as L
+        b, c, h, w = x.shape
+        y, code = _pool_out(x)
+        st = L.stream()
+        batch_stats = bn.training or bn.running_mean is None
+        if batch_stats:
+            ws = torch.empty(max(L.load().u2mkd_bn2d_workspace_bytes(b, c, h * w), 16), dtype=torch.uint8, device=x.device)
+            mean = torch.empty(c, dtype=torch.float32, device=x.device)
+            invstd = torch.empty_like(mean)
+            track = bn.training and bn.running_mean is not None
+            L.call('u2mkd_bn2d_pool_train_forward', L.ptr(x), b, c, h, w, L.ptr(weight), L.ptr(bias), bn.eps,
+                   bn.momentum if track else 0.0, L.ptr(bn.running_mean if track else None),
+                   L.ptr(bn.running_var if track else None), L.ptr(bn.num_batches_tracked if track else None),
+                   L.ptr(ws), L.ptr(mean), L.ptr(invstd), L.ptr(y), L.ptr(code), st)
+            if track:
+                torch._C._increment_version([t for t in (bn.running_mean, bn.running_var, bn.num_batches_tracked) if t is not None])
+        else:
+            mean, invstd = bn.running_mean, torch.rsqrt(bn.running_var + bn.eps)
+            L.call('u2mkd_bn2d_pool_eval_forward', L.ptr(x), b, c, h, w, L.ptr(weight), L.ptr(bias), bn.eps,
+                   L.ptr(bn.running_mean), L.ptr(bn.running_var), L.ptr(y), L.ptr(code), st)
+        ctx.save_for_backward(x, weight, bias, mean, invstd, code)
+        ctx.batch_stats = batch_stats
+        return y
+
+    @staticmethod
+    @torch.autograd.function.once_differentiable
+    def backward(ctx, g):
+        from . import _lib as L
+        x, weight, bias, mean, invstd, code = ctx.saved_tensors
+        b, c, h, w = x.shape
+        g = g.contiguous()
+        dx = torch.empty_like(x)
+        dgamma = torch.empty(c, dtype=torch.float32, device=x.device)
+        dbeta = torch.empty_like(dgamma)
+        ws = torch.empty(max(L.load().u2mkd_bn2d_workspace_bytes(b, c, h * w), 16), dtype=torch.uint8, device=x.device)
+        L.call('u2mkd_bn2d_pool_backward', L.ptr(g), L.ptr(code), L.ptr(x), b, c, h, w, L.ptr(mean), L.ptr(invstd),
+               L.ptr(weight), L.ptr(bias), int(ctx.batch_stats), L.ptr(ws), L.ptr(dgamma), L.ptr(dbeta), L.ptr(dx), L.stream())
+        return dx, (dgamma if weight is not None else None), (dbeta if bias is not None else None), None
+
+
+class _SyncBNReluPoolFunction(torch.autograd.Function):
+
+    @staticmethod
+    def forward(ctx, x, weight, bias, bn, group, world):
+        from . import _lib as L
+        from .torchsparse.nn.functional import _gather_rows, note_collective
+        b, c, h, w = x.shape
+        dev, st = x.device, L.stream()
+        ws = torch.empty(max(L.load().u2mkd_bn2d_workspace_bytes(b, c, h * w), 16), dtype=torch.uint8, device=dev)
+        stats = torch.empty(2 * c + 1, dtype=torch.float32, device=dev)
+        L.call('u2mkd_bn2d_local_stats', L.ptr(x), b, c, h * w, L.ptr(ws), L.ptr(stats), st)
+        note_collective('all_gather', stats)
+        if world > 1:
+            gathered = torch.empty(world, 2 * c + 1, dtype=torch.float32, device=dev)
+            _gather_rows(gathered, stats, group)
+        else:
+            gathered = stats.view(1, -1)
+        mit = torch.empty(2 * c + 1, dtype=torch.float32, device=dev)
+        mean, invstd, total = mit[:c], mit[c:2 * c], mit[2 * c:]
+        track = bn.running_mean is not None
+        L.call('u2mkd_bn_merge_stats', L.ptr(gathered), world, c, float(bn.eps), float(bn.momentum if track else 0.0),
+               L.ptr(bn.running_mean if track else None), L.ptr(bn.running_var if track else None), L.ptr(mean),
+               L.ptr(invstd), L.ptr(total), L.ptr(bn.num_batches_tracked if track else None), L.stream())
+        if track:
+            torch._C._increment_version([t for t in (bn.running_mean, bn.running_var, bn.num_batches_tracked) if t is not None])
+        y, code = _pool_out(x)
+        L.call('u2mkd_bn2d_pool_apply', L.ptr(x), b, c, h, w, L.ptr(mean), L.ptr(invstd), L.ptr(weight), L.ptr(bias),
+               L.ptr(y), L.ptr(code), L.stream())
+        ctx.save_for_backward(x, weight, bias, mean, invstd, total, code)
+        ctx.group, ctx.world = group, world
+        return y
+
+    @staticmethod
+    @torch.autograd.function.once_differentiable
+    def backward(ctx, g):
+        from . import _lib as L
+        from .torchsparse.nn.functional import _sum_over_ranks, note_collective
+        x, weight, bias, mean, invstd, total, code = ctx.saved_tensors
+        b, c, h, w = x.shape
+        g = g.contiguous()
+        dev = x.device
+        ws = torch.empty(max(L.load().u2mkd_bn2d_workspace_bytes(b, c, h * w), 16), dtype=torch.uint8, device=dev)
+        both = torch.empty(2, 2 * c, dtype=torch.float32, device=dev)
+        sums, local = both[0], both[1]
+        L.call('u2mkd_bn2d_pool_backward_local', L.ptr(g), L.ptr(code), L.ptr(x), b, c, h, w, L.ptr(mean), L.ptr(invstd),
+               L.ptr(weight), L.ptr(bias), L.ptr(ws), L.ptr(sums), L.ptr(local), L.stream())
+        note_collective('all_reduce', sums)
+        if ctx.world > 1:
+            _sum_over_ranks(sums, ctx.group)
+        dx = torch.empty_like(x)
+        L.call('u2mkd_bn2d_pool_backward_apply', L.ptr(g), L.ptr(code), L.ptr(x), b, c, h, w, L.ptr(total), L.ptr(mean),
+               L.ptr(invstd), L.ptr(weight), L.ptr(bias), L.ptr(sums), L.ptr(dx), L.stream())
+        return (dx, local[c:] if weight is not None else None, local[:c] if bias is not None else None, None, None, None)
+
+
+def bn_relu_pool(bn, pool, x):
+    if (_HIP_BN2D and isinstance(pool, MaxPool3x3s2) and isinstance(bn, (BatchNorm2d, SyncBatchNorm2d)) and x.is_cuda
+            and x.dtype == torch.float32 and x.dim() == 4 and x.is_contiguous() and x.numel() > 0 and not torch.is_autocast_enabled()
+            and x.shape[0] * x.shape[1] <= 65535 and x.shape[2] * x.shape[3] < 2 ** 30):
+        sync = None
+        if isinstance(bn, SyncBatchNorm2d) and bn.training:
+            from .torchsparse.nn.functional import _sync_group
+            sync = _sync_group(bn)
+        if sync is not None and bn.momentum is not None:
+            return _SyncBNReluPoolFunction.apply(x, bn.weight, bn.bias, bn, sync[0], sync[1])
+        if sync is None and (bn.momentum is not None or not bn.training):
+            return _BNReluPoolFunction.apply(x, bn.weight, bn.bias, bn)
+    return pool(bn_act(bn, x, relu=True))
 
 
 def bn_act(bn, x, relu=False, residual=None):
@@ -443,7 +563,7 @@
         return x, skip
 
     def forward_stem(self, image):
-        return self.maxpool(bn_act(self.bn1, self.conv1(image), relu=True))
+        return bn_relu_pool(self.bn1, self.maxpool, self.conv1(image))
 
     def forward_down(self, image):
         x = self.forward_stem(image)
diff --git a/u2mkd_amd/csrc/bn2d.hip b/u2mkd_amd/csrc/bn2d.hip
--- a/u2mkd_amd/csrc/bn2d.hip
+++ b/u2mkd_amd/csrc/bn2d.hip
@@ -1,4 +1,5 @@
 #include "common.h"
+#include "pool3s2.h"
 
 namespace u2mkd {
 
@@ -124,14 +125,78 @@
     }
 }
 
+__global__ void __launch_bounds__(256)
+bn2d_apply_pool_kernel(const float *__restrict__ x, int C, int h, int w, int oh, int ow, const float *__restrict__ mean,
+                       const float *__restrict__ invstd, const float *__restrict__ var, float eps,
+                       const float *__restrict__ gamma, const float *__restrict__ beta, float *__restrict__ y,
+                       uint8_t *__restrict__ code) {
+    const uint32_t pix = blockIdx.x * blockDim.x + threadIdx.x;
+    if (pix >= (uint32_t)(oh * ow)) return;
+    const int oy = (int)(pix / (uint32_t)ow), ox = (int)(pix - (uint32_t)oy * (uint32_t)ow);
+    const int64_t plane = blockIdx.y;
+    const int c = (int)(blockIdx.y % (uint32_t)C);
+    const float is = var ? 1.f / sqrtf(var[c] + eps) : invstd[c];
+    const float m = mean[c], g = gamma ? gamma[c] : 1.f, bt = beta ? beta[c] : 0.f;
+    float best;
+    int bc;
+    pool3s2_window_max(x + plane * (int64_t)h * w, h, w, oy, ox,
+                       [&](float v) {
+                           const float xh = (v - m) * is;
+                           const float o = xh * g + bt + 0.f;
+                           return fmaxf(o, 0.f);
+                       },
+                       best, bc);
+    const int64_t e = plane * oh * ow + pix;
+    y[e] = best;
+    code[e] = (uint8_t)bc;
+}
+
+struct B2Pool {
+    const uint8_t *code;
+    int w, oh, ow;
+};
+
+template <bool kPool> struct B2Grad;
+
+template <> struct B2Grad<false> {
+    const float *p;
+    __device__ B2Grad(const float *dy, const B2Pool &, size_t plane, int hw, int lo) : p(dy + plane * hw + lo) {}
+    __device__ __forceinline__ float at(int e) const { return p[e]; }
+    __device__ __forceinline__ float4 at4(int e) const { return *reinterpret_cast<const float4 *>(p + e); }
+};
+
+template <> struct B2Grad<true> {
+    const float *gp;
+    const uint8_t *cp;
+    int w, oh, ow, lo;
+    __device__ B2Grad(const float *g, const B2Pool &pool, size_t plane, int, int lo_)
+        : gp(g + plane * ((size_t)pool.oh * pool.ow)), cp(pool.code + plane * ((size_t)pool.oh * pool.ow)), w(pool.w),
+          oh(pool.oh), ow(pool.ow), lo(lo_) {}
+    __device__ __forceinline__ float at(int e) const {
+        const uint32_t q = (uint32_t)(lo + e);
+        const int yy = (int)(q / (uint32_t)w);
+        return pool3s2_gather(gp, cp, oh, ow, yy, (int)(q - (uint32_t)yy * (uint32_t)w));
+    }
+    __device__ __forceinline__ float4 at4(int e) const {
+        if ((w & 3) != 0) return make_float4(at(e), at(e + 1), at(e + 2), at(e + 3));
+        const uint32_t q = (uint32_t)(lo + e);
+        const int yy = (int)(q / (uint32_t)w);
+        float g[4];
+        pool3s2_gather4(gp, cp, oh, ow, yy, (int)(q - (uint32_t)yy * (uint32_t)w), g);
+        return make_float4(g[0], g[1], g[2], g[3]);
+    }
+};
+
+template <bool kPool>
 __global__ void __launch_bounds__(kB2Threads)
-bn2d_bwd_partial_kernel(const float *__restrict__ dy, const float *__restrict__ x, const float *__restrict__ res, int C,
-                        int hw, int splits, const float *__restrict__ mean, const float *__restrict__ invstd,
+bn2d_bwd_partial_kernel(const float *__restrict__ dy, B2Pool pool, const float *__restrict__ x, const float *__restrict__ res,
+                        int C, int hw, int splits, const float *__restrict__ mean, const float *__restrict__ invstd,
                         const float *__restrict__ gamma, const float *__restrict__ beta, int relu,
                         float *__restrict__ partial) {
     const int c = blockIdx.y, b = blockIdx.x / splits, s = blockIdx.x - b * splits;
     const int lo = s * kB2Chunk, cnt = min(kB2Chunk, hw - lo);
     const size_t base = ((size_t)b * C + c) * hw + lo;
+    const B2Grad<kPool> grad(dy, pool, (size_t)b * C + c, hw, lo);
     const float m = mean[c], is = invstd[c], g = gamma ? gamma[c] : 1.f, bt = beta ? beta[c] : 0.f;
     float s1 = 0.f, s2 = 0.f;
     auto one = [&](float v, float d, float r) {
@@ -143,12 +208,12 @@
     if ((hw & 3) == 0) {
         for (int e = threadIdx.x * 4; e < cnt; e += kB2Threads * 4) {
             const float4 v = *reinterpret_cast<const float4 *>(x + base + e);
-            const float4 d = *reinterpret_cast<const float4 *>(dy + base + e);
+            const float4 d = grad.at4(e);
             const float4 r = res ? *reinterpret_cast<const float4 *>(res + base + e) : make_float4(0.f, 0.f, 0.f, 0.f);
             one(v.x, d.x, r.x); one(v.y, d.y, r.y); one(v.z, d.z, r.z); one(v.w, d.w, r.w);
         }
     } else {
-        for (int e = threadIdx.x; e < cnt; e += kB2Threads) one(x[base + e], dy[base + e], (relu && res) ? res[base + e] : 0.f);
+        for (int e = threadIdx.x; e < cnt; e += kB2Threads) one(x[base + e], grad.at(e), (relu && res) ? res[base + e] : 0.f);
     }
     b2_block_sum2(s1, s2);
     if (threadIdx.x == 0) {
@@ -178,9 +243,10 @@
     }
 }
 
+template <bool kPool>
 __global__ void __launch_bounds__(kB2Threads)
-bn2d_bwd_apply_kernel(const float *__restrict__ dy, const float *__restrict__ x, const float *__restrict__ res, int C,
-                      int hw, int asplits, float inv_n, const float *__restrict__ mean, const float *__restrict__ invstd,
+bn2d_bwd_apply_kernel(const float *__restrict__ dy, B2Pool pool, const float *__restrict__ x, const float *__restrict__ res,
+                      int C, int hw, int asplits, float inv_n, const float *__restrict__ mean, const float *__restrict__ invstd,
                       const float *__restrict__ gamma, const float *__restrict__ beta, int relu,
                       const float *__restrict__ dbeta, const float *__restrict__ dgamma, float *__restrict__ dx,
                       float *__restrict__ dres, const float *__restrict__ total_n = nullptr) {
@@ -188,6 +254,7 @@
     const int c = blockIdx.y, b = blockIdx.x / asplits, s = blockIdx.x - b * asplits;
     const int lo = s * kB2ApplyChunk, cnt = min(kB2ApplyChunk, hw - lo);
     const size_t base = ((size_t)b * C + c) * hw + lo;
+    const B2Grad<kPool> grad(dy, pool, (size_t)b * C + c, hw, lo);
     const float m = mean[c], is = invstd[c], g = gamma ? gamma[c] : 1.f, bt = beta ? beta[c] : 0.f;
     const float k1 = dbeta ? dbeta[c] * inv_n : 0.f, k2 = dbeta ? dgamma[c] * inv_n : 0.f, gs = g * is;
     auto one = [&](float v, float d, float r, float &dm) {
@@ -199,7 +266,7 @@
     if ((hw & 3) == 0) {
         for (int e = threadIdx.x * 4; e < cnt; e += kB2Threads * 4) {
             const float4 v = *reinterpret_cast<const float4 *>(x + base + e);
-            const float4 d = *reinterpret_cast<const float4 *>(dy + base + e);
+            const float4 d = grad.at4(e);
             const float4 r = (relu && res) ? *reinterpret_cast<const float4 *>(res + base + e) : make_float4(0.f, 0.f, 0.f, 0.f);
             float4 o, dm;
             o.x = one(v.x, d.x, r.x, dm.x); o.y = one(v.y, d.y, r.y, dm.y);
@@ -210,7 +277,7 @@
     } else {
         for (int e = threadIdx.x; e < cnt; e += kB2Threads) {
             float dm;
-            dx[base + e] = one(x[base + e], dy[base + e], (relu && res) ? res[base + e] : 0.f, dm);
+            dx[base + e] = one(x[base + e], grad.at(e), (relu && res) ? res[base + e] : 0.f, dm);
             if (dres) dres[base + e] = dm;
         }
     }
@@ -269,12 +336,12 @@
     U2_REQUIRE(b2_shape_ok(b, c, hw), "u2mkd_bn2d_backward: shape [%lld, %d, %lld] out of range", (long long)b, c, (long long)hw);
     const int splits = b2_splits((int)hw, kB2Chunk), asplits = b2_splits((int)hw, kB2ApplyChunk);
     float *partial = reinterpret_cast<float *>(workspace);
-    hipLaunchKernelGGL(bn2d_bwd_partial_kernel, dim3((unsigned)(splits * b), (unsigned)c), dim3(kB2Threads), 0, as_stream(s), dy, x,
-                       res, c, (int)hw, splits, mean, invstd, gamma, beta, relu, partial);
+    hipLaunchKernelGGL(bn2d_bwd_partial_kernel<false>, dim3((unsigned)(splits * b), (unsigned)c), dim3(kB2Threads), 0, as_stream(s), dy,
+                       B2Pool{}, x, res, c, (int)hw, splits, mean, invstd, gamma, beta, relu, partial);
     hipLaunchKernelGGL(bn2d_bwd_finalize_kernel, dim3((unsigned)c), dim3(64), 0, as_stream(s), partial, (int)(splits * b), dbeta,
                        dgamma);
-    hipLaunchKernelGGL(bn2d_bwd_apply_kernel, dim3((unsigned)(asplits * b), (unsigned)c), dim3(kB2Threads), 0, as_stream(s), dy, x,
-                       res, c, (int)hw, asplits, 1.f / (float)(b * hw), mean, invstd, gamma, beta, relu, batch_stats ? dbeta : nullptr,
+    hipLaunchKernelGGL(bn2d_bwd_apply_kernel<false>, dim3((unsigned)(asplits * b), (unsigned)c), dim3(kB2Threads), 0, as_stream(s), dy,
+                       B2Pool{}, x, res, c, (int)hw, asplits, 1.f / (float)(b * hw), mean, invstd, gamma, beta, relu, batch_stats ? dbeta : nullptr,
                        batch_stats ? dgamma : nullptr, dx, dres);
     return check_launch("u2mkd_bn2d_backward");
 }
@@ -312,8 +379,8 @@
     U2_REQUIRE(b2_shape_ok(b, c, hw), "u2mkd_bn2d_backward_local: shape [%lld, %d, %lld] out of range", (long long)b, c, (long long)hw);
     const int splits = b2_splits((int)hw, kB2Chunk);
     float *partial = reinterpret_cast<float *>(workspace);
-    hipLaunchKernelGGL(bn2d_bwd_partial_kernel, dim3((unsigned)(splits * b), (unsigned)c), dim3(kB2Threads), 0, as_stream(s), dy, x,
-                       res, c, (int)hw, splits, mean, invstd, gamma, beta, relu, partial);
+    hipLaunchKernelGGL(bn2d_bwd_partial_kernel<false>, dim3((unsigned)(splits * b), (unsigned)c), dim3(kB2Threads), 0, as_stream(s), dy,
+                       B2Pool{}, x, res, c, (int)hw, splits, mean, invstd, gamma, beta, relu, partial);
     hipLaunchKernelGGL(bn2d_bwd_finalize_kernel, dim3((unsigned)c), dim3(64), 0, as_stream(s), partial, (int)(splits * b), sums,
                        sums + c, keep);
     return check_launch("u2mkd_bn2d_backward_local");
@@ -326,9 +393,110 @@
     U2_REQUIRE(dy && x && total_n && mean && invstd && sums && dx, "u2mkd_bn2d_backward_apply: null pointer");
     U2_REQUIRE(b2_shape_ok(b, c, hw), "u2mkd_bn2d_backward_apply: shape [%lld, %d, %lld] out of range", (long long)b, c, (long long)hw);
     const int asplits = b2_splits((int)hw, kB2ApplyChunk);
-    hipLaunchKernelGGL(bn2d_bwd_apply_kernel, dim3((unsigned)(asplits * b), (unsigned)c), dim3(kB2Threads), 0, as_stream(s), dy, x,
-                       res, c, (int)hw, asplits, 0.f, mean, invstd, gamma, beta, relu, sums, sums + c, dx, dres, total_n);
+    hipLaunchKernelGGL(bn2d_bwd_apply_kernel<false>, dim3((unsigned)(asplits * b), (unsigned)c), dim3(kB2Threads), 0, as_stream(s), dy,
+                       B2Pool{}, x, res, c, (int)hw, asplits, 0.f, mean, invstd, gamma, beta, relu, sums, sums + c, dx, dres, total_n);
     return check_launch("u2mkd_bn2d_backward_apply");
 }
 
-}
+#define B2_POOL_REQUIRE(name)                                                                                               \
+    U2_REQUIRE(h > 0 && w > 0 && b2_shape_ok(b, c, (int64_t)h * w) && b * c <= 65535,                                      \
+               name ": shape [%lld, %d, %d, %d] out of range (at most 65535 planes)", (long long)b, c, h, w)
+
+static void b2_launch_apply_pool(const float *x, int64_t b, int32_t c, int32_t h, int32_t w, const float *mean,
+                                 const float *invstd, const float *var, float eps, const float *gamma, const float *beta,
+                                 float *y, uint8_t *code, u2mkd_stream_t s) {
+    const int oh = pool3s2_out(h), ow = pool3s2_out(w);
+    hipLaunchKernelGGL(bn2d_apply_pool_kernel, dim3((unsigned)ceil_div((int64_t)oh * ow, 256), (unsigned)(b * c)), dim3(256), 0,
+                       as_stream(s), x, c, h, w, oh, ow, mean, invstd, var, eps, gamma, beta, y, code);
+}
+
+static void b2_launch_pool_bwd_partial(const float *g, const uint8_t *code, const float *x, int64_t b, int32_t c, int32_t h,
+                                       int32_t w, const float *mean, const float *invstd, const float *gamma,
+                                       const float *beta, float *partial, u2mkd_stream_t s) {
+    const int hw = h * w, splits = b2_splits(hw, kB2Chunk);
+    hipLaunchKernelGGL(bn2d_bwd_partial_kernel<true>, dim3((unsigned)(splits * b), (unsigned)c), dim3(kB2Threads), 0, as_stream(s), g,
+                       B2Pool{code, w, pool3s2_out(h), pool3s2_out(w)}, x, (const float *)nullptr, c, hw, splits, mean, invstd,
+                       gamma, beta, 1, partial);
+}
+
+static void b2_launch_pool_bwd_apply(const float *g, const uint8_t *code, const float *x, int64_t b, int32_t c, int32_t h,
+                                     int32_t w, float inv_n, const float *total_n, const float *mean, const float *invstd,
+                                     const float *gamma, const float *beta, const float *dbeta, const float *dgamma, float *dx,
+                                     u2mkd_stream_t s) {
+    const int hw = h * w, asplits = b2_splits(hw, kB2ApplyChunk);
+    hipLaunchKernelGGL(bn2d_bwd_apply_kernel<true>, dim3((unsigned)(asplits * b), (unsigned)c), dim3(kB2Threads), 0, as_stream(s), g,
+                       B2Pool{code, w, pool3s2_out(h), pool3s2_out(w)}, x, (const float *)nullptr, c, hw, asplits, inv_n, mean,
+                       invstd, gamma, beta, 1, dbeta, dgamma, dx, (float *)nullptr, total_n);
+}
+
+int u2mkd_bn2d_pool_train_forward(const float *x, int64_t b, int32_t c, int32_t h, int32_t w, const float *gamma,
+                                  const float *beta, float eps, float momentum, float *running_mean, float *running_var,
+                                  int64_t *num_batches_tracked, void *workspace, float *mean, float *invstd, float *y,
+                                  uint8_t *code, u2mkd_stream_t s) {
+    U2_REQUIRE(x && workspace && mean && invstd && y && code, "u2mkd_bn2d_pool_train_forward: null pointer");
+    B2_POOL_REQUIRE("u2mkd_bn2d_pool_train_forward");
+    const int64_t hw = (int64_t)h * w;
+    U2_REQUIRE(b * hw > 1, "u2mkd_bn2d_pool_train_forward: more than one value per channel is needed in training mode");
+    const int splits = b2_splits((int)hw, kB2Chunk);
+    float *partial = reinterpret_cast<float *>(workspace);
+    hipLaunchKernelGGL(bn2d_stats_partial_kernel, dim3((unsigned)(splits * b), (unsigned)c), dim3(kB2Threads), 0, as_stream(s), x,
+                       c, (int)hw, splits, partial);
+    hipLaunchKernelGGL(bn2d_stats_finalize_kernel, dim3((unsigned)c), dim3(64), 0, as_stream(s), partial, (int)(splits * b),
+                       (int)hw, splits, eps, momentum, running_mean, running_var, num_batches_tracked, mean, invstd);
+    b2_launch_apply_pool(x, b, c, h, w, mean, invstd, nullptr, eps, gamma, beta, y, code, s);
+    return check_launch("u2mkd_bn2d_pool_train_forward");
+}
+
+int u2mkd_bn2d_pool_eval_forward(const float *x, int64_t b, int32_t c, int32_t h, int32_t w, const float *gamma,
+                                 const float *beta, float eps, const float *running_mean, const float *running_var, float *y,
+                                 uint8_t *code, u2mkd_stream_t s) {
+    U2_REQUIRE(x && running_mean && running_var && y && code, "u2mkd_bn2d_pool_eval_forward: null pointer");
+    B2_POOL_REQUIRE("u2mkd_bn2d_pool_eval_forward");
+    b2_launch_apply_pool(x, b, c, h, w, running_mean, nullptr, running_var, eps, gamma, beta, y, code, s);
+    return check_launch("u2mkd_bn2d_pool_eval_forward");
+}
+
+int u2mkd_bn2d_pool_apply(const float *x, int64_t b, int32_t c, int32_t h, int32_t w, const float *mean, const float *invstd,
+                          const float *gamma, const float *beta, float *y, uint8_t *code, u2mkd_stream_t s) {
+    U2_REQUIRE(x && mean && invstd && y && code, "u2mkd_bn2d_pool_apply: null pointer");
+    B2_POOL_REQUIRE("u2mkd_bn2d_pool_apply");
+    b2_launch_apply_pool(x, b, c, h, w, mean, invstd, nullptr, 0.f, gamma, beta, y, code, s);
+    return check_launch("u2mkd_bn2d_pool_apply");
+}
+
+int u2mkd_bn2d_pool_backward(const float *g, const uint8_t *code, const float *x, int64_t b, int32_t c, int32_t h, int32_t w,
+                             const float *mean, const float *invstd, const float *gamma, const float *beta,
+                             int32_t batch_stats, void *workspace, float *dgamma, float *dbeta, float *dx, u2mkd_stream_t s) {
+    U2_REQUIRE(g && code && x && mean && invstd && workspace && dgamma && dbeta && dx, "u2mkd_bn2d_pool_backward: null pointer");
+    B2_POOL_REQUIRE("u2mkd_bn2d_pool_backward");
+    float *partial = reinterpret_cast<float *>(workspace);
+    b2_launch_pool_bwd_partial(g, code, x, b, c, h, w, mean, invstd, gamma, beta, partial, s);
+    hipLaunchKernelGGL(bn2d_bwd_finalize_kernel, dim3((unsigned)c), dim3(64), 0, as_stream(s), partial,
+                       (int)(b2_splits(h * w, kB2Chunk) * b), dbeta, dgamma);
+    b2_launch_pool_bwd_apply(g, code, x, b, c, h, w, 1.f / (float)(b * h * w), nullptr, mean, invstd, gamma, beta,
+                             batch_stats ? dbeta : nullptr, batch_stats ? dgamma : nullptr, dx, s);
+    return check_launch("u2mkd_bn2d_pool_backward");
+}
+
+int u2mkd_bn2d_pool_backward_local(const float *g, const uint8_t *code, const float *x, int64_t b, int32_t c, int32_t h,
+                                   int32_t w, const float *mean, const float *invstd, const float *gamma, const float *beta,
+                                   void *workspace, float *sums, float *keep, u2mkd_stream_t s) {
+    U2_REQUIRE(g && code && x && mean && invstd && workspace && sums, "u2mkd_bn2d_pool_backward_local: null pointer");
+    B2_POOL_REQUIRE("u2mkd_bn2d_pool_backward_local");
+    float *partial = reinterpret_cast<float *>(workspace);
+    b2_launch_pool_bwd_partial(g, code, x, b, c, h, w, mean, invstd, gamma, beta, partial, s);
+    hipLaunchKernelGGL(bn2d_bwd_finalize_kernel, dim3((unsigned)c), dim3(64), 0, as_stream(s), partial,
+                       (int)(b2_splits(h * w, kB2Chunk) * b), sums, sums + c, keep);
+    return check_launch("u2mkd_bn2d_pool_backward_local");
+}
+
+int u2mkd_bn2d_pool_backward_apply(const float *g, const uint8_t *code, const float *x, int64_t b, int32_t c, int32_t h,
+                                   int32_t w, const float *total_n, const float *mean, const float *invstd,
+                                   const float *gamma, const float *beta, const float *sums, float *dx, u2mkd_stream_t s) {
+    U2_REQUIRE(g && code && x && total_n && mean && invstd && sums && dx, "u2mkd_bn2d_pool_backward_apply: null pointer");
+    B2_POOL_REQUIRE("u2mkd_bn2d_pool_backward_apply");
+    b2_launch_pool_bwd_apply(g, code, x, b, c, h, w, 0.f, total_n, mean, invstd, gamma, beta, sums, sums + c, dx, s);
+    return check_launch("u2mkd_bn2d_pool_backward_apply");
+}
+
+}
diff --git a/u2mkd_amd/csrc/pixhead.hip b/u2mkd_amd/csrc/pixhead.hip
--- a/u2mkd_amd/csrc/pixhead.hip
+++ b/u2mkd_amd/csrc/pixhead.hip
@@ -1,4 +1,5 @@
 #include "common.h"
+#include "pool3s2.h"
 
 namespace u2mkd {
 
@@ -211,23 +212,9 @@
     const int oy = (int)(pix / (uint32_t)ow), ox = (int)(pix - (uint32_t)oy * (uint32_t)ow);
     const int64_t plane = blockIdx.y;
     const int64_t e = plane * oh * ow + pix;
-    const float *xp = x + plane * (int64_t)h * w;
-    const int y0 = 2 * oy - 1, x0 = 2 * ox - 1;
-    float best = -INFINITY;
-    int bc = 0;
-    bool first = true;
-#pragma unroll
-    for (int dy = 0; dy < 3; ++dy) {
-        const int yy = y0 + dy;
-        if (yy < 0 || yy >= h) continue;
-#pragma unroll
-        for (int dx = 0; dx < 3; ++dx) {
-            const int xx = x0 + dx;
-            if (xx < 0 || xx >= w) continue;
-            const float v = xp[(int64_t)yy * w + xx];
-            if (first || v > best || v != v) { best = v; bc = dy * 3 + dx; first = false; }
-        }
-    }
+    float best;
+    int bc;
+    pool3s2_window_max(x + plane * (int64_t)h * w, h, w, oy, ox, [](float v) { return v; }, best, bc);
     y[e] = best;
     code[e] = (uint8_t)bc;
 }
@@ -240,24 +227,7 @@
     const int yy = (int)(pix / (uint32_t)w), xx = (int)(pix - (uint32_t)yy * (uint32_t)w);
     const int64_t plane = blockIdx.y;
     const int64_t e = plane * h * w + pix;
-    const float *gp = dy + plane * (int64_t)oh * ow;
-    const uint8_t *cp = code + plane * (int64_t)oh * ow;
-    float g = 0.f;
-    const int oy0 = yy >> 1, oy1 = (yy + 1) >> 1, ox0 = xx >> 1, ox1 = (xx + 1) >> 1;
-#pragma unroll
-    for (int a = 0; a < 2; ++a) {
-        const int oy = a ? oy1 : oy0;
-        if ((a && oy1 == oy0) || oy >= oh) continue;
-        const int dyw = yy - (2 * oy - 1);
-#pragma unroll
-        for (int b = 0; b < 2; ++b) {
-            const int ox = b ? ox1 : ox0;
-            if ((b && ox1 == ox0) || ox >= ow) continue;
-            const int dxw = xx - (2 * ox - 1);
-            if (cp[(int64_t)oy * ow + ox] == dyw * 3 + dxw) g += gp[(int64_t)oy * ow + ox];
-        }
-    }
-    dx[e] = g;
+    dx[e] = pool3s2_gather(dy + plane * (int64_t)oh * ow, code + plane * (int64_t)oh * ow, oh, ow, yy, xx);
 }
 
 __global__ void __launch_bounds__(256)
diff --git a/u2mkd_amd/csrc/pool3s2.h b/u2mkd_amd/csrc/pool3s2.h
--- /dev/null
+++ b/u2mkd_amd/csrc/pool3s2.h
@@ -0,0 +1,92 @@
+#pragma once
+#include "common.h"
+
+namespace u2mkd {
+
+__host__ __device__ inline int pool3s2_out(int n) { return (n + 2 - 3) / 2 + 1; }
+
+template <class F>
+__device__ __forceinline__ void pool3s2_window_max(const float *__restrict__ xp, int h, int w, int oy, int ox, F f,
+                                                   float &best, int &bc) {
+    const int y0 = 2 * oy - 1, x0 = 2 * ox - 1;
+    float v[9];
+#pragma unroll
+    for (int dy = 0; dy < 3; ++dy)
+#pragma unroll
+        for (int dx = 0; dx < 3; ++dx)
+            v[dy * 3 + dx] = xp[(int64_t)min(max(y0 + dy, 0), h - 1) * w + min(max(x0 + dx, 0), w - 1)];
+    best = -INFINITY;
+    bc = 0;
+    bool first = true;
+#pragma unroll
+    for (int dy = 0; dy < 3; ++dy) {
+#pragma unroll
+        for (int dx = 0; dx < 3; ++dx) {
+            const bool inside = y0 + dy >= 0 && y0 + dy < h && x0 + dx >= 0 && x0 + dx < w;
+            const float u = f(v[dy * 3 + dx]);
+            if (inside && (first || u > best || u != u)) { best = u; bc = dy * 3 + dx; first = false; }
+        }
+    }
+}
+
+__device__ __forceinline__ float pool3s2_gather(const float *__restrict__ gp, const uint8_t *__restrict__ cp, int oh, int ow,
+                                                int yy, int xx) {
+    const int oy0 = yy >> 1, oy1 = (yy + 1) >> 1, ox0 = xx >> 1, ox1 = (xx + 1) >> 1;
+    int code[4];
+    float v[4];
+#pragma unroll
+    for (int a = 0; a < 2; ++a)
+#pragma unroll
+        for (int b = 0; b < 2; ++b) {
+            const int64_t at = (int64_t)min(a ? oy1 : oy0, oh - 1) * ow + min(b ? ox1 : ox0, ow - 1);
+            code[a * 2 + b] = cp[at];
+            v[a * 2 + b] = gp[at];
+        }
+    float g = 0.f;
+#pragma unroll
+    for (int a = 0; a < 2; ++a) {
+        const int oy = a ? oy1 : oy0;
+        const int dyw = yy - (2 * oy - 1);
+#pragma unroll
+        for (int b = 0; b < 2; ++b) {
+            const int ox = b ? ox1 : ox0;
+            const int dxw = xx - (2 * ox - 1);
+            const bool window = !(a && oy1 == oy0) && oy < oh && !(b && ox1 == ox0) && ox < ow;
+            if (window && code[a * 2 + b] == dyw * 3 + dxw) g += v[a * 2 + b];
+        }
+    }
+    return g;
+}
+
+__device__ __forceinline__ void pool3s2_gather4(const float *__restrict__ gp, const uint8_t *__restrict__ cp, int oh, int ow,
+                                                int yy, int x0, float (&g)[4]) {
+    const int oy0 = yy >> 1, oy1 = (yy + 1) >> 1, oxb = x0 >> 1;
+    int code[6];
+    float v[6];
+#pragma unroll
+    for (int a = 0; a < 2; ++a)
+#pragma unroll
+        for (int b = 0; b < 3; ++b) {
+            const int64_t at = (int64_t)min(a ? oy1 : oy0, oh - 1) * ow + min(oxb + b, ow - 1);
+            code[a * 3 + b] = cp[at];
+            v[a * 3 + b] = gp[at];
+        }
+    g[0] = g[1] = g[2] = g[3] = 0.f;
+#pragma unroll
+    for (int a = 0; a < 2; ++a) {
+        const int oy = a ? oy1 : oy0;
+        const bool row = !(a && oy1 == oy0) && oy < oh;
+        const int dyw = yy - (2 * oy - 1);
+#pragma unroll
+        for (int b = 0; b < 3; ++b) {
+            const int ox = oxb + b;
+            const int sel = code[a * 3 + b] - 3 * dyw;
+            const int col = 2 * ox - 1 + sel - x0;
+            const bool window = row && ox < ow && sel >= 0 && sel < 3;
+#pragma unroll
+            for (int i = 0; i < 4; ++i) g[i] += (window && col == i) ? v[a * 3 + b] : 0.f;
+        }
+    }
+}
+
+}
```

Measured after the change: 1.181 million. 1.5% lower.
